# zalgo3/zfista

Hardware: AMD Instinct MI355X
Metric: fista_iterations_per_sec_n1e8_per_gpu_shard (higher is better)
Workload: dtype f64

## Files before the change

### include/zfista_hip.h

```cpp
#ifndef ZFISTA_HIP_H
#define ZFISTA_HIP_H

#include <stdint.h>

#ifdef __cplusplus
extern "C" {
#endif

#define ZF_ABI_VERSION 7

#define ZF_OK 0
#define ZF_ERR_HIP (-1)
#define ZF_ERR_ARG (-2)
#define ZF_ERR_STATE (-3)
#define ZF_ERR_NODEVICE (-4)

#define ZF_RUNNING 0
#define ZF_CONVERGED 1
#define ZF_MAXITER 2
#define ZF_BACKTRACK_FAILED 3

#define ZF_PROBLEM_DIAG_QUAD_L1 1
#define ZF_PROBLEM_LEAST_SQUARES_L1 2
#define ZF_PROBLEM_BLUR_HAAR_L1 3
// ... 71 lines not shown
    double lr;
    double tol;
    double tol_internal;
    double decay_rate;
    int64_t max_iter;
    int64_t max_backtrack_iter;
    int32_t nesterov;
    int32_t deprecated;
    int32_t sub_iters;
    int32_t accept_mode;
} zf_options;

typedef struct zf_solver zf_solver;

int zf_abi_version(void);
const char* zf_last_error(void);
int64_t zf_sizeof_control(void);
int zf_device_count(int* count);
int zf_set_device(int device);
int zf_malloc(void** dev_ptr, int64_t bytes);
int zf_free(void* dev_ptr);
int zf_memcpy_h2d(void* dst_dev, const void* src_host, int64_t bytes, void* stream);
int zf_memcpy_d2h(void* dst_host, const void* src_dev, int64_t bytes, void* stream);
int zf_memcpy_d2d(void* dst_dev, const void* src_dev, int64_t bytes, void* stream);
int zf_stream_synchronize(void* stream);
int zf_shutdown(void);

typedef struct zf_comm zf_comm;
int zf_comm_unique_id(void* id128);
int zf_comm_create(zf_comm** out, int32_t rank, int32_t world, const void* id128);
int zf_comm_destroy(zf_comm* c);
int zf_comm_create_local_group(zf_comm** out_world, int32_t world, int64_t cap_doubles);
int zf_comm_info(zf_comm* c, int32_t* rank, int32_t* world);
typedef struct zf_comm_desc {
    int32_t rank, world;
    int32_t kind;
    int32_t nccl_count;
    int32_t nccl_user_rank;
    int32_t nccl_device;
    int32_t rccl_version;
    int32_t reserved;
    int64_t all_gathers;
    char library[256];
} zf_comm_desc;
int zf_comm_describe(zf_comm* c, zf_comm_desc* out, int64_t out_bytes);
int zf_comm_all_gather(zf_comm* c, const double* send_dev, double* recv_dev, int64_t count, void* stream);

int zf_op_eval(const double* taps_dev, int32_t k, const double* b_dev, int64_t h, int64_t w, double scale,
               const double* x_host, double* f_out, double* grad_out_host);

int zf_decide_host(zf_control* ctl, int64_t ctl_bytes , const double* packs,
                   double* trace);

int zf_solver_create(zf_solver** out, const zf_problem_desc* desc, const zf_options* opt,
                     void* stream);
int zf_solver_destroy(zf_solver* s);
int zf_solver_enqueue_init(zf_solver* s, const double* x0_dev);
int zf_solver_enqueue_init_commit(zf_solver* s);
int zf_solver_set_beta(zf_solver* s, int64_t first, const double* beta_host, int64_t count);
int zf_solver_enqueue_steps(zf_solver* s, int64_t steps);
int zf_solver_autotune(zf_solver* s, int32_t* chosen_tiles);
int zf_solver_flush(zf_solver* s);
int zf_solver_set_comm(zf_solver* s, zf_comm* comm);
int zf_solver_enqueue_init_all(zf_solver* s, const double* x0_dev);
int zf_solver_enqueue_trial(zf_solver* s);
int zf_solver_enqueue_decide(zf_solver* s);
int zf_solver_sub_iters(zf_solver* s, int32_t* sub_iters);
int zf_solver_set_history(zf_solver* s, double* hist_dev, int64_t cap_slots, int64_t stride);
int zf_solver_set_max_iter(zf_solver* s, int64_t max_iter);
int zf_solver_pack_ptrs(zf_solver* s, double** pack_local_dev, double** pack_all_dev);
int zf_solver_set_pack_buffers(zf_solver* s, double* pack_local_dev, double* pack_all_dev);
int zf_solver_svec_ptrs(zf_solver* s, double** s_part_dev, double** s_all_dev);
int zf_solver_set_svec_buffers(zf_solver* s, double* s_part_dev, double* s_all_dev);
int zf_solver_enqueue_trial_finish(zf_solver* s);
int zf_solver_enqueue_init_finish(zf_solver* s);
int zf_solver_poll(zf_solver* s, zf_control* ctl_host, int64_t ctl_bytes, double* trace_host, int64_t trace_bytes);
int zf_solver_x_dev(zf_solver* s, const double** x_dev);
int zf_solver_get_x(zf_solver* s, double* x_host, int64_t count );
int zf_solver_get_x_prev(zf_solver* s, double* x_host, int64_t count );
int zf_solver_restore(zf_solver* s, const double* xk_dev, const double* xprev_dev, const zf_control* saved,
                      int64_t saved_bytes );
int zf_solver_trial_kernel_ms(zf_solver* s, double* avg_ms, int64_t* launches);
int zf_solver_launch_counts(zf_solver* s, int64_t* out, int64_t count );
int zf_solver_ls_plan(zf_solver* s, int64_t* out, int64_t count );
int zf_solver_pass_stats(zf_solver* s, double* out, int64_t count );
int zf_solver_pass_stats_ex(zf_solver* s, double* out, int64_t count );
int zf_solver_exchange_stats(zf_solver* s, double* out, int64_t count );
int zf_solver_pass_records(zf_solver* s, double* out, int64_t cap_pairs, int64_t* count);
int zf_solver_set_timing(zf_solver* s, int32_t enabled);

int zf_host_grad_step(double* v_host, const double* y_host, const double* jac_host, double lr,
                      int64_t n);
int zf_host_model_terms(const double* jac_host, const double* x_host, const double* y_host,
                        int64_t n, double out3[3]);
int zf_host_momentum(double* y_out_host, const double* x_host, const double* x_old_host,
                     double beta, int64_t n);
int zf_dev_grad_step(double* v_dev, const double* y_dev, const double* jac_dev, double lr, int64_t n, void* stream);
int zf_dev_model_terms(const double* jac_dev, const double* x_dev, const double* y_dev, int64_t n,
                       double out3_host[3], void* stream);
int zf_dev_model_terms_async(const double* jac_dev, const double* x_dev, const double* y_dev, int64_t n,
                             double* out3_dev, void* stream);
int zf_dev_momentum(double* y_out_dev, const double* x_dev, const double* x_old_dev, double beta, int64_t n,
                    void* stream);
int zf_dev_mo_combine(double* v_dev, const double* y_dev, const double* J_dev, const double* w_host, double lr,
                      int32_t m, int64_t n, double* ss_dev, void* stream);
int zf_dev_mo_post_terms(const double* J_dev, const double* y_dev, const double* p_dev, const double* v_dev,
                         int32_t m, int64_t n, double* out_dev , void* stream);

int zf_host_prox_l1_box(double* out_host, const double* x_host, double tau, double lo, double hi,
                        int64_t n);
int zf_host_asum(const double* x_host, int64_t n, double* out);
int zf_host_diag_grad(double* out_host, const double* x_host, const double* d_dev,
                      const double* c_dev, int64_t n);
int zf_ls_remainder_eval(const double* s_plus_host, const double* s_k_host, const double* s_km1_host, int64_t m, double beta,
                         int32_t nesterov, double scale, int32_t wide, double* r_out);

typedef struct zf_spmv_plan {
    int32_t lanes;
    int32_t reserved;
    int64_t threshold;
    int64_t nsplit;
    int64_t nseg;
    const int64_t* split_row;
    const int64_t* split_first;
    const int64_t* seg_start;
} zf_spmv_plan;
typedef struct zf_spmat zf_spmat;
int zf_spmat_create(zf_spmat** out, int64_t m, int64_t n, int64_t nnz, const int64_t* indptr_dev, const int32_t* indices_dev,
                    const double* values_dev, const zf_spmv_plan* plan, const int64_t* t_indptr_dev, const int32_t* t_indices_dev,
                    const double* t_values_dev, const zf_spmv_plan* t_plan, int64_t plan_bytes);
int zf_spmat_destroy(zf_spmat* h);
int zf_solver_create_sparse(zf_solver** out, const zf_problem_desc* desc, const zf_spmat* h, const zf_options* opt, void* stream);

int zf_solver_create_sparse_responses(zf_solver** out, const zf_problem_desc* desc, const zf_spmat* h, int32_t K, const zf_options* opt,
                                      void* stream);
int zf_spmat_mr_apply(const zf_spmat* h, int32_t transpose, int32_t K, double out_scale, const double* in_host, double* out_host);

int zf_solver_duality_gap(zf_solver* s, double* out, int64_t count );


int zf_solver_set_l2(zf_solver* s, double l2);
int zf_host_prox_enet_box(double* out_host, const double* x_host, double tau, double shrink, double lo, double hi, int64_t n);
int zf_host_enet_g(const double* x_host, int64_t n, double lam, double l2, double* out);

int zf_spmat_col_norms(const zf_spmat* h, double* norms_dev, double* stats_dev);
int zf_dense_col_norms(const double* A_dev, int64_t m_rows, int64_t n, double* norms_dev, double* stats_dev);
int zf_screen_scan(const uint8_t* keep_dev, int64_t n, int32_t* index_dev, int64_t* count_out);
int zf_spmat_restrict_count(const zf_spmat* h, const uint8_t* keep_dev, int32_t* index_dev, int64_t* len_dev, int64_t* t_len_dev,
                            int32_t* seg_off_dev, int64_t* count_out);
int zf_spmat_restrict_fill(const zf_spmat* h, const uint8_t* keep_dev, const int32_t* index_dev, const int32_t* seg_off_dev, int64_t k,
                           int64_t nnz_new, const int64_t* indptr_dev, int32_t* indices_dev, double* values_dev,
                           const int64_t* t_indptr_dev, int32_t* t_indices_dev, double* t_values_dev);
int zf_dense_restrict(const double* A_dev, int64_t m_rows, int64_t n, const uint8_t* keep_dev, int32_t* index_dev, int64_t k,
                      double* out_dev);

int zf_solver_set_huber(zf_solver* s, double delta);

enum { ZF_LOSS_SQUARE = 0, ZF_LOSS_LOGISTIC = 1, ZF_LOSS_HUBER = 2 };
int zf_solver_set_row_weights(zf_solver* s, const double* w_dev);

enum { ZF_LOSS_POISSON = 3 };
int zf_solver_set_poisson(zf_solver* s);

int zf_solver_set_penalty_factors(zf_solver* s, const double* p_dev);
int zf_host_prox_pf_box(double* out_host, const double* x_host, const double* p_host, double t, double lo, double hi, int64_t n);
int zf_host_pf_g(const double* x_host, const double* p_host, int64_t n, double lam, double* out);
// ... 87 lines not shown
```

### zfista_amd/_lib.py

```python
from __future__ import annotations

import ctypes as C
import os
import subprocess

import numpy as np

_HERE = os.path.dirname(os.path.abspath(__file__))
CSRC = os.path.join(_HERE, "csrc")
LIB_PATH = os.environ.get("ZF_LIB_PATH") or os.path.join(CSRC, "libzfista_hip.so")

ZF_OK = 0
ZF_RUNNING, ZF_CONVERGED, ZF_MAXITER, ZF_BACKTRACK_FAILED = 0, 1, 2, 3
ZF_PROBLEM_DIAG_QUAD_L1, ZF_PROBLEM_LEAST_SQUARES_L1, ZF_PROBLEM_BLUR_HAAR_L1 = 1, 2, 3
ZF_PROBLEM_SPARSE_LS_L1 = 4
ZF_PROBLEM_LOGISTIC_L1, ZF_PROBLEM_SPARSE_LOGISTIC_L1 = 5, 6
ZF_LOSS_SQUARE, ZF_LOSS_LOGISTIC, ZF_LOSS_HUBER, ZF_LOSS_POISSON, ZF_LOSS_MULTINOMIAL = 0, 1, 2, 3, 4
ZF_MO_GENERIC, ZF_MO_JOS1, ZF_MO_FDS = 0, 1, 2
ZF_PACK_LEN, ZF_TRACE_COLS, ZF_RING = 8, 8, 1024
ZF_MAX_SUB_ITERS = 16
ZF_MAX_LAG = 2 * ZF_MAX_SUB_ITERS - 2
ZF_PEND_FLUSH = -1
TR_ERR, TR_F, TR_LR, TR_FUN, TR_TRIALS, TR_FX, TR_GX, TR_FY = range(8)
PK_FY, PK_DOT, PK_SS, PK_GX, PK_FX, PK_ERR = range(6)
# ... 49 lines not shown
class CommDesc(C.Structure):

    _fields_ = [
        ("rank", C.c_int32), ("world", C.c_int32), ("kind", C.c_int32), ("nccl_count", C.c_int32),
        ("nccl_user_rank", C.c_int32), ("nccl_device", C.c_int32), ("rccl_version", C.c_int32), ("reserved", C.c_int32),
        ("all_gathers", C.c_int64), ("library", C.c_char * 256),
    ]


class SpmvPlan(C.Structure):

    _fields_ = [
        ("lanes", C.c_int32), ("reserved", C.c_int32), ("threshold", C.c_int64), ("nsplit", C.c_int64), ("nseg", C.c_int64),
        ("split_row", C.c_void_p), ("split_first", C.c_void_p), ("seg_start", C.c_void_p),
    ]


class EvalDesc(C.Structure):

    _fields_ = [
        ("A", C.c_void_p), ("A32", C.c_void_p), ("spmat", C.c_void_p), ("m_rows", C.c_int64), ("n", C.c_int64),
        ("b", C.c_void_p), ("w", C.c_void_p), ("p", C.c_void_p),
        ("scale", C.c_double), ("lam", C.c_double), ("l2", C.c_double), ("delta", C.c_double),
        ("loss", C.c_int32), ("K", C.c_int32),
    ]


_P = C.c_void_p
_D = C.POINTER(C.c_double)
SIGNATURES = {
    "zf_abi_version": (C.c_int, []),
    "zf_last_error": (C.c_char_p, []),
    "zf_sizeof_control": (C.c_int64, []),
    "zf_device_count": (C.c_int, [C.POINTER(C.c_int)]),
    "zf_set_device": (C.c_int, [C.c_int]),
    "zf_malloc": (C.c_int, [C.POINTER(_P), C.c_int64]),
    "zf_free": (C.c_int, [_P]),
    "zf_memcpy_h2d": (C.c_int, [_P, _P, C.c_int64, _P]),
    "zf_memcpy_d2h": (C.c_int, [_P, _P, C.c_int64, _P]),
    "zf_memcpy_d2d": (C.c_int, [_P, _P, C.c_int64, _P]),
    "zf_stream_synchronize": (C.c_int, [_P]),
    "zf_shutdown": (C.c_int, []),
    "zf_comm_unique_id": (C.c_int, [_P]),
    "zf_comm_create": (C.c_int, [C.POINTER(_P), C.c_int32, C.c_int32, _P]),
    "zf_comm_destroy": (C.c_int, [_P]),
    "zf_comm_create_local_group": (C.c_int, [C.POINTER(_P), C.c_int32, C.c_int64]),
    "zf_comm_info": (C.c_int, [_P, C.POINTER(C.c_int32), C.POINTER(C.c_int32)]),
    "zf_comm_describe": (C.c_int, [_P, C.POINTER(CommDesc), C.c_int64]),
    "zf_comm_all_gather": (C.c_int, [_P, _P, _P, C.c_int64, _P]),
    "zf_solver_set_comm": (C.c_int, [_P, _P]),
    "zf_solver_enqueue_init_all": (C.c_int, [_P, _P]),
    "zf_decide_host": (C.c_int, [C.POINTER(Control), C.c_int64, _P, _P]),
    "zf_solver_create": (C.c_int, [C.POINTER(_P), C.POINTER(ProblemDesc), C.POINTER(Options), _P]),
    "zf_solver_destroy": (C.c_int, [_P]),
    "zf_solver_enqueue_init": (C.c_int, [_P, _P]),
    "zf_solver_enqueue_init_commit": (C.c_int, [_P]),
    "zf_solver_set_beta": (C.c_int, [_P, C.c_int64, _P, C.c_int64]),
    "zf_solver_enqueue_steps": (C.c_int, [_P, C.c_int64]),
    "zf_solver_autotune": (C.c_int, [_P, C.POINTER(C.c_int32)]),
    "zf_solver_flush": (C.c_int, [_P]),
    "zf_solver_enqueue_trial": (C.c_int, [_P]),
    "zf_solver_enqueue_decide": (C.c_int, [_P]),
    "zf_solver_sub_iters": (C.c_int, [_P, C.POINTER(C.c_int32)]),
    "zf_solver_set_history": (C.c_int, [_P, _P, C.c_int64, C.c_int64]),
    "zf_solver_set_max_iter": (C.c_int, [_P, C.c_int64]),
    "zf_solver_pack_ptrs": (C.c_int, [_P, C.POINTER(_P), C.POINTER(_P)]),
    "zf_solver_set_pack_buffers": (C.c_int, [_P, _P, _P]),
    "zf_solver_svec_ptrs": (C.c_int, [_P, C.POINTER(_P), C.POINTER(_P)]),
    "zf_solver_set_svec_buffers": (C.c_int, [_P, _P, _P]),
    "zf_solver_enqueue_trial_finish": (C.c_int, [_P]),
    "zf_solver_enqueue_init_finish": (C.c_int, [_P]),
    "zf_solver_poll": (C.c_int, [_P, C.POINTER(Control), C.c_int64, _P, C.c_int64]),
    "zf_solver_x_dev": (C.c_int, [_P, C.POINTER(_P)]),
    "zf_solver_get_x": (C.c_int, [_P, _P, C.c_int64]),
    "zf_solver_get_x_prev": (C.c_int, [_P, _P, C.c_int64]),
    "zf_solver_restore": (C.c_int, [_P, _P, _P, C.POINTER(Control), C.c_int64]),
    "zf_solver_trial_kernel_ms": (C.c_int, [_P, C.POINTER(C.c_double), C.POINTER(C.c_int64)]),
    "zf_solver_set_timing": (C.c_int, [_P, C.c_int32]),
    "zf_solver_pass_stats": (C.c_int, [_P, _P, C.c_int64]),
    "zf_solver_pass_stats_ex": (C.c_int, [_P, _P, C.c_int64]),
    "zf_solver_exchange_stats": (C.c_int, [_P, _P, C.c_int64]),
    "zf_solver_pass_records": (C.c_int, [_P, _P, C.c_int64, C.POINTER(C.c_int64)]),
    "zf_solver_launch_counts": (C.c_int, [_P, _P, C.c_int64]),
    "zf_solver_ls_plan": (C.c_int, [_P, _P, C.c_int64]),
    "zf_host_grad_step": (C.c_int, [_P, _P, _P, C.c_double, C.c_int64]),
    "zf_host_model_terms": (C.c_int, [_P, _P, _P, C.c_int64, _P]),
    "zf_host_momentum": (C.c_int, [_P, _P, _P, C.c_double, C.c_int64]),
    "zf_dev_grad_step": (C.c_int, [_P, _P, _P, C.c_double, C.c_int64, _P]),
    "zf_dev_model_terms": (C.c_int, [_P, _P, _P, C.c_int64, _P, _P]),
    "zf_dev_model_terms_async": (C.c_int, [_P, _P, _P, C.c_int64, _P, _P]),
    "zf_dev_momentum": (C.c_int, [_P, _P, _P, C.c_double, C.c_int64, _P]),
    "zf_dev_mo_combine": (C.c_int, [_P, _P, _P, _P, C.c_double, C.c_int32, C.c_int64, _P, _P]),
    "zf_dev_mo_post_terms": (C.c_int, [_P, _P, _P, _P, C.c_int32, C.c_int64, _P, _P]),
    "zf_eval_diag_l1": (C.c_int, [_P, _P, _P, C.c_double, C.c_int64, _P, _P]),
    "zf_host_prox_l1_box": (C.c_int, [_P, _P, C.c_double, C.c_double, C.c_double, C.c_int64]),
    "zf_host_asum": (C.c_int, [_P, C.c_int64, C.POINTER(C.c_double)]),
    "zf_host_diag_grad": (C.c_int, [_P, _P, _P, _P, C.c_int64]),
    "zf_mo_create": (C.c_int, [C.POINTER(_P), C.c_int32, C.c_int32, C.c_int64, _P, _P, C.c_double, C.c_double, _P]),
    "zf_mo_set_shard": (C.c_int, [_P, C.c_int64, C.c_int64, _P, _P]),
    "zf_mo_set_comm": (C.c_int, [_P, _P, C.c_int64, C.c_int64]),
    "zf_mo_exchange_count": (C.c_int, [_P, C.POINTER(C.c_int64)]),
    "zf_mo_set_bounds": (C.c_int, [_P, _P, _P]),
    "zf_mo_destroy": (C.c_int, [_P]),
    "zf_mo_set_x0": (C.c_int, [_P, _P]),
    "zf_mo_eval_F": (C.c_int, [_P, C.c_int32, _P, _P]),
    "zf_mo_prepare": (C.c_int, [_P, _P]),
    "zf_mo_set_jac": (C.c_int, [_P, _P]),
    "zf_mo_dual_eval": (C.c_int, [_P, C.c_double, _P, _P]),
    "zf_mo_dual_hessian": (C.c_int, [_P, C.c_double, _P, _P]),
    "zf_mo_solve_dual": (C.c_int, [_P, C.c_double, _P, _P, C.c_int32, _P, C.c_double, C.c_int64, _P,
                                  C.POINTER(C.c_double), C.POINTER(C.c_int64), C.POINTER(C.c_int32),
                                  C.POINTER(C.c_int64)]),
    "zf_mo_solve_dual_stream": (C.c_int, [_P, C.c_double, _P, _P, C.c_int32, _P, C.c_double, C.c_int64, _P,
                                         C.POINTER(C.c_double), C.POINTER(C.c_int64), C.POINTER(C.c_int32),
                                         C.POINTER(C.c_int64)]),
    "zf_mo_solve_dual_device": (C.c_int, [_P, C.c_double, _P, _P, C.c_int32, _P, C.c_double, C.c_int64, _P,
                                         C.POINTER(C.c_double), C.POINTER(C.c_int64), C.POINTER(C.c_int32),
                                         C.POINTER(C.c_int64), C.POINTER(C.c_double), _P, _P, _P]),
    "zf_mo_prepare_async": (C.c_int, [_P]),
    "zf_mo_set_fused": (C.c_int, [_P, C.c_int32]),
    "zf_mo_trial_launch": (C.c_int, [_P, C.c_double, _P, C.c_int32, _P, C.c_double, C.c_int64, C.c_double, C.c_int32,
                                     C.c_int32, _P]),
    "zf_mo_trial_wait": (C.c_int, [_P, C.c_int32, _P, _P, _P, _P, _P, _P, _P, _P, _P, _P, _P]),
    "zf_mo_uncommit": (C.c_int, [_P]),
    "zf_mo_invalidate_prepare": (C.c_int, [_P, C.c_int32]),
    "zf_mo_debug_force_timeout": (C.c_int, [_P, C.c_int32]),
    "zf_mo_get_f_y": (C.c_int, [_P, _P]),
    "zf_mo_solve_stats": (C.c_int, [_P, _P, C.c_int64]),
    "zf_mo_recover": (C.c_int, [_P, C.c_double, _P, _P]),
    "zf_mo_commit": (C.c_int, [_P, C.c_double, C.c_int32]),
    "zf_mo_get": (C.c_int, [_P, C.c_int32, _P, C.c_int64]),
    "zf_mo_put": (C.c_int, [_P, C.c_int32, _P]),
    "zf_mo_get_jac": (C.c_int, [_P, _P, C.c_int64]),
    "zf_mo_prox_host": (C.c_int, [_P, _P, _P, _P]),
    "zf_mo_post_terms": (C.c_int, [_P, C.c_double, _P, _P, _P]),
    "zf_op_eval": (C.c_int, [_P, C.c_int32, _P, C.c_int64, C.c_int64, C.c_double, _P, C.POINTER(C.c_double), _P]),
    "zf_ls_remainder_eval": (C.c_int, [_P, _P, _P, C.c_int64, C.c_double, C.c_int32, C.c_double, C.c_int32, C.POINTER(C.c_double)]),
    "zf_spmat_create": (C.c_int, [C.POINTER(_P), C.c_int64, C.c_int64, C.c_int64, _P, _P, _P, C.POINTER(SpmvPlan),
                                  _P, _P, _P, C.POINTER(SpmvPlan), C.c_int64]),
    "zf_spmat_destroy": (C.c_int, [_P]),
    "zf_solver_duality_gap": (C.c_int, [_P, _P, C.c_int64]),
    "zf_solver_create_sparse": (C.c_int, [C.POINTER(_P), C.POINTER(ProblemDesc), _P, C.POINTER(Options), _P]),
    "zf_spmat_col_norms": (C.c_int, [_P, _P, _P]),
    "zf_dense_col_norms": (C.c_int, [_P, C.c_int64, C.c_int64, _P, _P]),
    "zf_screen_scan": (C.c_int, [_P, C.c_int64, _P, C.POINTER(C.c_int64)]),
    "zf_spmat_restrict_count": (C.c_int, [_P, _P, _P, _P, _P, _P, C.POINTER(C.c_int64)]),
    "zf_spmat_restrict_fill": (C.c_int, [_P, _P, _P, _P, C.c_int64, C.c_int64, _P, _P, _P, _P, _P, _P]),
    "zf_dense_restrict": (C.c_int, [_P, C.c_int64, C.c_int64, _P, _P, C.c_int64, _P]),
    "zf_solver_set_l2": (C.c_int, [_P, C.c_double]),
    "zf_host_prox_enet_box": (C.c_int, [_P, _P, C.c_double, C.c_double, C.c_double, C.c_double, C.c_int64]),
    "zf_host_enet_g": (C.c_int, [_P, C.c_int64, C.c_double, C.c_double, C.POINTER(C.c_double)]),
    "zf_solver_set_huber": (C.c_int, [_P, C.c_double]),
    "zf_solver_set_row_weights": (C.c_int, [_P, _P]),
    "zf_solver_set_poisson": (C.c_int, [_P]),
    "zf_solver_set_multinomial": (C.c_int, [_P]),
    "zf_solver_set_penalty_factors": (C.c_int, [_P, _P]),
    "zf_host_prox_pf_box": (C.c_int, [_P, _P, _P, C.c_double, C.c_double, C.c_double, C.c_int64]),
    "zf_host_pf_g": (C.c_int, [_P, _P, C.c_int64, C.c_double, C.POINTER(C.c_double)]),
    "zf_solver_set_matrix_f32": (C.c_int, [_P, _P]),
    "zf_solver_set_responses": (C.c_int, [_P, C.c_int32]),
    "zf_solver_create_sparse_responses": (C.c_int, [C.POINTER(_P), C.POINTER(ProblemDesc), _P, C.c_int32, C.POINTER(Options), _P]),
    "zf_spmat_mr_apply": (C.c_int, [_P, C.c_int32, C.c_int32, C.c_double, _P, _P]),
    "zf_sizeof_eval_desc": (C.c_int64, []),
    "zf_margins_eval": (C.c_int, [C.POINTER(EvalDesc), C.c_int64, _P, C.POINTER(C.c_double), _P]),
    "zf_margins_gap": (C.c_int, [C.POINTER(EvalDesc), C.c_int64, _P, _P, C.c_int64]),
    "zf_margins_screen": (C.c_int, [C.POINTER(EvalDesc), C.c_int64, _P, _P, C.c_int64, _P, _P, C.c_int64, C.c_int64, _P, _P]),
}

_lib = None


def build(verbose: bool = False) -> str:
    out = subprocess.run(["make", "-C", CSRC], capture_output=True, text=True)
    if out.returncode != 0:
        raise HipUnavailable(f"building libzfista_hip.so failed:\n{out.stdout}\n{out.stderr}")
    if verbose:
        print(out.stdout)
    return LIB_PATH


def load():
    global _lib
    if _lib is not None:
        return _lib
    if not os.path.exists(LIB_PATH):
        raise HipUnavailable(
            f"{LIB_PATH} is not built; run `make -C {CSRC}` (or __graft_entry__.build()). "
            "zfista_amd has no CPU fallback."
        )
    try:
        import torch
    except Exception:
        pass
    try:
        lib = C.CDLL(LIB_PATH)
    except OSError as exc:
        raise HipUnavailable(f"cannot load {LIB_PATH}: {exc}") from exc
    for name, (res, args) in SIGNATURES.items():
        fn = getattr(lib, name)
        fn.restype = res
        fn.argtypes = args
    if lib.zf_sizeof_control() != C.sizeof(Control):
        raise HipUnavailable("zf_control layout mismatch between library and Python mirror")
    if lib.zf_sizeof_eval_desc() != C.sizeof(EvalDesc):
        raise HipUnavailable("zf_eval_desc layout mismatch between library and Python mirror")
    _lib = lib
    return lib


def check(rc: int, what: str = ""):
    if rc != ZF_OK:
        msg = load().zf_last_error().decode(errors="replace")
        raise ZfError(f"{what or 'libzfista_hip'} failed ({rc}): {msg}")


def require_gpu():
    lib = load()
    n = C.c_int(0)
    rc = lib.zf_device_count(C.byref(n))
    if rc != ZF_OK or n.value < 1:
        raise HipUnavailable(
            "no usable GPU: " + lib.zf_last_error().decode(errors="replace")
            + " - zfista_amd runs its solver arithmetic on MI355X only (no CPU fallback)."
        )
    return lib


ENV_SWITCHES = ("ZF_SPECULATE", "ZF_LS_SMALL", "ZF_GEMV_MFMA", "ZF_TILES_PER_WG", "ZF_SUB_ITERS",
                "ZF_COMM", "ZF_MO_COMM", "ZF_MO_LAUNCH_AHEAD", "ZF_MO_SPIN_LIMIT", "ZF_RCCL_LIB", "ZF_DUAL_SOLVER",
                "ZF_FORCE_SPLIT", "ZF_LIB_PATH", "ZF_BENCH_BACKEND",
                "ZF_RUNAHEAD", "ZF_RUNAHEAD_SPIN_LIMIT", "ZF_PASS_SEQ_START", "ZF_AHEAD",
                "ZF_AHEAD_UNSHARDED", "ZF_ACCEPT", "ZF_OP_SEPARABLE", "ZF_OP_FUSE_PROX", "ZF_OP_PERSIST", "ZF_RUNAHEAD_SHARDED")


def env_overrides() -> dict:
    return {k: os.environ[k] for k in ENV_SWITCHES if k in os.environ}


def ptr(a: np.ndarray) -> int:
    return a.ctypes.data
```

### zfista_amd/csrc/zf_common.h

```cpp
#pragma once
#include <hip/hip_runtime.h>
#include <stdint.h>
#include <stdio.h>
#include <string.h>

#include "../../include/zfista_hip.h"

extern thread_local char zf_errbuf[512];
static inline int zf_fail(int code, const char* fmt, const char* a = "", const char* b = "") {
    snprintf(zf_errbuf, sizeof(zf_errbuf), fmt, a, b);
    return code;
}
#define ZF_HIP(expr)                                                                   \
    do {                                                                               \
        hipError_t _e = (expr);                                                        \
        if (_e != hipSuccess) return zf_fail(ZF_ERR_HIP, "%s: %s", #expr, hipGetErrorString(_e)); \
    } while (0)
#define ZF_REQUIRE(cond, msg)                                  \
    do {                                                       \
        if (!(cond)) return zf_fail(ZF_ERR_ARG, "%s%s", msg);  \
    } while (0)

struct zf_env {
    bool speculate;
    int pass_seq_start;
    int sub_iters;
    bool runahead;
    int tiles_per_wg;
    unsigned runahead_spin;
    int runahead_sharded;
    bool ahead;
    bool ahead_unsharded;
    bool gemv_mfma;
    bool ls_small;
    bool op_separable;
    bool op_fuse_prox;
    bool op_persist;
    long long mo_spin_limit;
};
zf_env zf_env_read();

constexpr int ZF_BLOCK = 256;
constexpr int ZF_MAX_GRID = 2048;
constexpr int ZF_WAVES = ZF_BLOCK / 64;

static inline int zf_grid_for(int64_t items_per_thread_units) {
    int64_t blocks = (items_per_thread_units + ZF_BLOCK - 1) / ZF_BLOCK;
    if (blocks < 1) blocks = 1;
    if (blocks > ZF_MAX_GRID) blocks = ZF_MAX_GRID;
    return (int)blocks;
}

__device__ __forceinline__ void zf_publish(double* p, double v) {
    __hip_atomic_store(p, v, __ATOMIC_RELAXED, __HIP_MEMORY_SCOPE_AGENT);
}
__device__ __forceinline__ double zf_consume(const double* p) {
    return __hip_atomic_load(p, __ATOMIC_RELAXED, __HIP_MEMORY_SCOPE_AGENT);
}

__device__ __forceinline__ double zf_wave_sum(double v) {
#pragma unroll
    for (int off = 32; off > 0; off >>= 1) v += __shfl_down(v, off, 64);
    return v;
}
__device__ __forceinline__ double zf_wave_max(double v) {
#pragma unroll
    for (int off = 32; off > 0; off >>= 1) v = fmax(v, __shfl_down(v, off, 64));
    return v;
}

template <int NS, int NM, int WAVES>
__device__ __forceinline__ void zf_block_reduce(const double (&sums)[NS], const double (&maxs)[NM > 0 ? NM : 1],
                                                double* lds , double& out) {
    const int lane = threadIdx.x & 63, wave = threadIdx.x >> 6;
#pragma unroll
    for (int k = 0; k < NS; ++k) {
        double v = zf_wave_sum(sums[k]);
        if (lane == 0) lds[wave * (NS + NM) + k] = v;
    }
#pragma unroll
    for (int k = 0; k < NM; ++k) {
        double v = zf_wave_max(maxs[k]);
        if (lane == 0) lds[wave * (NS + NM) + NS + k] = v;
    }
    __syncthreads();
    if (threadIdx.x < NS + NM) {
        const int k = threadIdx.x;
        double v = lds[k];
        if (k < NS) {
            for (int w = 1; w < WAVES; ++w) v += lds[w * (NS + NM) + k];
        } else {
            for (int w = 1; w < WAVES; ++w) v = fmax(v, lds[w * (NS + NM) + k]);
        }
        out = v;
    }
}

template <int N, int H, bool IS_MAX, int LVL>
__device__ __forceinline__ void zf_wave_reduce_multi_level(double (&v)[N], int lane) {
    if constexpr (LVL < 6) {
        constexpr int off = 32 >> LVL;
        if constexpr (LVL < H) {
            constexpr int half = N >> (LVL + 1);
            const bool hi = (lane & off) != 0;
#pragma unroll
            for (int q = 0; q < half; ++q) {
                const double send = hi ? v[q] : v[q + half];
                const double keep = hi ? v[q + half] : v[q];
                const double recv = __shfl_xor(send, off, 64);
                v[q] = IS_MAX ? fmax(keep, recv) : keep + recv;
            }
        } else {
            constexpr int cnt = N >> H;
#pragma unroll
            for (int q = 0; q < cnt; ++q) {
                const double recv = __shfl_xor(v[q], off, 64);
                v[q] = IS_MAX ? fmax(v[q], recv) : v[q] + recv;
            }
        }
        zf_wave_reduce_multi_level<N, H, IS_MAX, LVL + 1>(v, lane);
    }
// ... 38 lines not shown
```

### zfista_amd/csrc/zf_kernels_step.h

```cpp
#pragma once
#include <type_traits>

#include "zf_common.h"
#include "zf_decide.h"

constexpr int ZF_NPART = 6;

struct zf_elem_acc {
    double fy, dot, ss, l1, fx, mx;
};

template <bool NESTEROV, bool BOX, bool RES = false>
__device__ __forceinline__ double zf_elem_diag(double xk, double xo, double d, double c, double beta,
                                               double lr, double tau, double lo, double hi,
                                               zf_elem_acc& a) {
    double y = xk;
    if (NESTEROV) y = xk + beta * (xk - xo);
    const double r = y - c;
    const double grad = d * r;
    a.fy = __builtin_fma(grad, r, a.fy);
    const double v = y - lr * grad;
    double xn = zf_soft_threshold_nn(v, tau);
    if (BOX) xn = zf_clip(xn, lo, hi);
    const double dx = xn - y;
// ... 112 lines not shown
                     : "=&s"(keep) : "v"(gsrc), "s"(lds_dst) : "memory");
    else
        asm volatile("s_mov_b32 %0, m0\n\ts_mov_b32 m0, %2\n\ts_nop 0\n\tglobal_load_lds_dwordx4 %1, off\n\ts_mov_b32 m0, %0"
                     : "=&s"(keep) : "v"(gsrc), "s"(lds_dst) : "memory");
}
template <int N> __device__ __forceinline__ void zf_wait_vm() {
    asm volatile("s_waitcnt vmcnt(%0)" ::"n"(N) : "memory");
}
typedef __attribute__((address_space(3))) void* zf_lds_ptr;
#ifndef ZF_S16_GLDS
#define ZF_S16_GLDS 1
#endif
#ifndef ZF_S8_GLDS
#define ZF_S8_GLDS 0
#endif
#ifndef ZF_GENERAL_SINGLE_LOOP
#define ZF_GENERAL_SINGLE_LOOP 1
#endif
#ifndef ZF_GLDS_STAGES
#define ZF_GLDS_STAGES 3
#endif
#ifndef ZF_MID_REG_MAX
#define ZF_MID_REG_MAX 10
#endif
template <int S, int MODE, bool HIST, bool GRAD_INLINE, int SP = S> constexpr bool zf_uses_glds() {
    if (HIST || !GRAD_INLINE || ZF_S16_GLDS == 0) return false;
    if (S >= 16) return true;
    if (MODE == 0 && SP >= 16 && S > ZF_MID_REG_MAX) return true;
    if (ZF_S8_GLDS == 2) return S == 8 && SP >= 16 && MODE == 1;
    return ZF_S8_GLDS != 0 && S == 8 && SP >= 16;
}
constexpr int ZF_GLDS_STREAMS = 4;
constexpr int ZF_GLDS_STAGE_UNITS = ZF_GLDS_STREAMS * ZF_BLOCK;
constexpr int ZF_GLDS_NST = ZF_GLDS_STAGES;
static_assert(ZF_GLDS_NST >= 2 && ZF_GLDS_NST <= 4, "2 .. 4 stages");

constexpr int ZF_MAX_SUB = ZF_MAX_SUB_ITERS;
constexpr int zf_chain_h(int S) {
    int h = 0;
    while (h < 4 && S % (2 << h) == 0) ++h;
    return h;
}
constexpr int ZF_MID_MIN = 9;
constexpr int ZF_MID_MAX = 15;
ZF_HD inline int zf_pass_part(int S, int lag, int nf) {
    if (lag == 0 && nf == S) return 0;
#ifndef ZF_MID_CHAIN_OFF
    if (S >= 16 && lag == 0 && nf >= ZF_MID_MIN && nf <= ZF_MID_MAX) return 3;
#endif
    if (S >= 16 && nf > S / 2) return 2;
    return 1;
}
ZF_HD inline bool zf_pass_claims(int PART, int L, int S, int lag, int nf) {
    if (PART == 0) return lag == 0 && nf == S;
    if (PART == 3) return lag == 0 && nf == L;
    const bool longer = S >= 16 && nf > S / 2 && !(lag == 0 && nf == S);
    return PART == 2 ? longer : !longer && !(lag == 0 && nf == S);
}
#ifndef ZF_S16_UB
#define ZF_S16_UB 1
#endif
constexpr int ZF_MAX_RING = 6;

struct zf_pass_head {
    int cur, prev, ring;
    double lr, beta_next;
    int64_t nit;
};


struct zf_step_args {
    const zf_control* ctl;
    const double* beta_ring;
    double* xb[ZF_MAX_RING];
    const double* p0;
    const double* p1;
    double lam, lo, hi;
    int64_t n;
    int tiles_per_wg;
    double* blk_part;
    int* pass_log;
    int pass_slot;
    int pass_tag;
    double* hist;
    int64_t hist_cap;
    int64_t hist_stride;
    int fin_mode;
    int fin_gsz, fin_ng;
    double* grp_part;
    unsigned* fin_cnt;
    double fin_scale_f, fin_scale_g;
    double* pack;
    zf_control* ctl_rw;
    int decide;
    double* trace;
    int pass_seq;
    int fb_on, fb_part, fb_len;
    unsigned long long* ra_word;
    unsigned* ra_flags;
    int ra_wait;
    int ra_need;
    unsigned ra_spin;
    zf_pass_head ra_head;
    unsigned* ra_stats;
    double head_stamp;
    int head_nf;
    int fin_grid;
    int accept_mode;
};

ZF_HD inline int zf_log_shape(int lag, int nf, int passes) { return (nf & 31) | ((lag & 31) << 5) | ((passes & 63) << 10); }

struct zf_finalize_args {
    const double* blk_part;
    int nblocks;
    int sub_iters;
    double* slice_part;
    unsigned* cnt;
    double scale[ZF_NPART];
    const double* f_y_ext;
    const double* f_x_ext;
    const double* r_ext;
    int contribute_f;
    int contribute_x;
    double* pack;
    zf_control* ctl;
    int decide;
    double* trace;
    const double* beta_ring;
};

template <int S>
__global__ __launch_bounds__(ZF_FIN_THREADS) void zf_finalize_kernel(zf_finalize_args F) {
    constexpr int NQ = S * ZF_NPART;
    constexpr int NW = ZF_FIN_THREADS / 64;
    __shared__ double lds[NW * NQ];
    __shared__ zf_trial_eval s_pre[ZF_MAX_SUB_ITERS];
    __shared__ double s_pack[ZF_MAX_SUB_ITERS * ZF_PACK_LEN];
    __shared__ double s_single[NQ];
    __shared__ int s_last;
    if (F.ctl->status != ZF_RUNNING) return;
    const int lane = threadIdx.x & 63, wave = threadIdx.x >> 6;
    const int per = (F.nblocks + (int)gridDim.x - 1) / (int)gridDim.x;
    const int b0 = blockIdx.x * per;
    int b1 = b0 + per;
    if (b1 > F.nblocks) b1 = F.nblocks;
    constexpr int GT = S < 8 ? S : 8;
    constexpr int GH = zf_chain_h(GT);
#pragma unroll
    for (int j0 = 0; j0 < S; j0 += GT) {
        double sums[5 * GT], maxs[GT];
#pragma unroll
        for (int k = 0; k < 5 * GT; ++k) sums[k] = 0.0;
#pragma unroll
        for (int k = 0; k < GT; ++k) maxs[k] = 0.0;
        for (int b = b0 + threadIdx.x; b < b1; b += ZF_FIN_THREADS) {
            double p[ZF_NPART * GT];
#pragma unroll
            for (int k = 0; k < ZF_NPART * GT; ++k) p[k] = F.blk_part[(int64_t)(j0 * ZF_NPART + k) * F.nblocks + b];
#pragma unroll
            for (int j = 0; j < GT; ++j) {
#pragma unroll
                for (int k = 0; k < 5; ++k) sums[j * 5 + k] = sums[j * 5 + k] + p[j * ZF_NPART + k];
                maxs[j] = fmax(maxs[j], p[j * ZF_NPART + 5]);
            }
        }
        zf_wave_reduce_multi<5 * GT, GH, false>(sums, lane);
        zf_wave_reduce_multi<GT, GH, true>(maxs, lane);
        if ((lane & ((64 >> GH) - 1)) == 0) {
#pragma unroll
            for (int q = 0; q < 5; ++q) {
                const int idx = zf_wave_reduce_multi_index<5 * GT, GH>(q, lane);
                lds[wave * NQ + (j0 + idx / 5) * ZF_NPART + idx % 5] = sums[q];
            }
            lds[wave * NQ + (j0 + zf_wave_reduce_multi_index<GT, GH>(0, lane)) * ZF_NPART + 5] = maxs[0];
        }
    }
    __syncthreads();
    const bool single = (gridDim.x == 1);
    if (threadIdx.x < NQ) {
        const int k = threadIdx.x;
        double r = lds[k];
        for (int w = 1; w < NW; ++w)
            r = (k % ZF_NPART == ZF_NPART - 1) ? fmax(r, lds[w * NQ + k]) : r + lds[w * NQ + k];
        if (single) s_single[k] = r;
        else zf_publish(F.slice_part + (int64_t)k * ZF_FIN_WGS + blockIdx.x, r);
    }
    if (single) {
        if (threadIdx.x == 0) s_last = 1;
    } else {
        asm volatile("s_waitcnt vmcnt(0)" ::: "memory");
        if (NQ > 64) __syncthreads();
        if (threadIdx.x == 0) {
            const unsigned t = __hip_atomic_fetch_add(F.cnt, 1u, __ATOMIC_RELAXED, __HIP_MEMORY_SCOPE_AGENT);
// ... 106 lines not shown
    }
    __syncthreads();
    if (s_role == 0) return;
    auto sum_rows = [&](const double* rows, int count) -> double {
        double acc = 0.0, comp = 0.0;
        auto add = [&](double p) {
            if (is_max) {
                acc = fmax(acc, p);
            } else {
                const double tsum = acc + p;
                comp += (fabs(acc) >= fabs(p)) ? (acc - tsum) + p : (p - tsum) + acc;
                acc = tsum;
            }
        };
        if (count > 32 && count <= 64) {
            double p[64];
#pragma unroll
            for (int u = 0; u < 64; ++u) p[u] = (u < count) ? zf_consume(rows + (int64_t)u * NQ) : 0.0;
#pragma unroll
            for (int u = 0; u < 64; ++u) add(p[u]);
            return is_max ? acc : acc + comp;
        }
        for (int k0 = 0; k0 < count; k0 += 32) {
            double p[32];
#pragma unroll
            for (int u = 0; u < 32; ++u) p[u] = (k0 + u < count) ? zf_consume(rows + (int64_t)(k0 + u) * NQ) : 0.0;
#pragma unroll
            for (int u = 0; u < 32; ++u) add(p[u]);
        }
        return is_max ? acc : acc + comp;
    };
    if (s_role == 1) {
        const int g = b / gsz, b0 = g * gsz;
        const int b1 = b0 + gsz <= G ? b0 + gsz : G;
        if (t < NQ) zf_publish(A.grp_part + (int64_t)g * NQ + t, sum_rows(A.blk_part + (int64_t)b0 * NQ + t, b1 - b0));
        asm volatile("s_waitcnt vmcnt(0)" ::: "memory");
        __syncthreads();
        if (t == 0) {
            const unsigned tk = __hip_atomic_fetch_add(A.fin_cnt, 1u, __ATOMIC_RELAXED, __HIP_MEMORY_SCOPE_AGENT);
            const int last = (tk == (unsigned)(ng - 1));
            if (last) __hip_atomic_store(A.fin_cnt, 0u, __ATOMIC_RELAXED, __HIP_MEMORY_SCOPE_AGENT);
            asm volatile("s_waitcnt vmcnt(0)" ::: "memory");
            s_role = last ? 2 : 0;
        }
        __syncthreads();
        if (s_role != 2) return;
    }
    if (t < NQ) s_tot[t] = grouped ? sum_rows(A.grp_part + t, ng) : sum_rows(A.blk_part + t, G);
    __syncthreads();
    if (t >= 64) return;
    constexpr int SH = zf_chain_h(SP);
    constexpr int LSTR = 64 >> SH;
    const int trial = t / LSTR;
    const double* q = s_tot + trial * ZF_NPART;
    double pk[ZF_PACK_LEN];
    pk[ZF_PK_FY] = A.fin_scale_f * q[0];
    pk[ZF_PK_DOT] = q[1];
    pk[ZF_PK_SS] = q[2];
    pk[ZF_PK_GX] = A.fin_scale_g * q[3];
    pk[ZF_PK_FX] = A.fin_scale_f * q[4];
    pk[ZF_PK_ERR] = q[5];
    pk[7] = 0.0;
    if (A.accept_mode != 0) {
        pk[7] = pk[ZF_PK_FX];
        pk[ZF_PK_FX] = pk[ZF_PK_FY] + pk[7];
    }
    pk[6] = A.decide ? 0.0 : zf_pack_stamp(A.ctl_rw);
    if constexpr (RA) {
        if (!A.decide) {
            const bool poisoned = __hip_atomic_load(A.ra_flags + G + (A.pass_seq & 3), __ATOMIC_RELAXED, __HIP_MEMORY_SCOPE_AGENT) == (unsigned)A.pass_seq;
            pk[6] = poisoned ? 0.0 : A.head_stamp;
        }
    }
    if (t % LSTR == 0) {
#pragma unroll
        for (int k = 0; k < ZF_PACK_LEN; ++k) {
            A.pack[trial * ZF_PACK_LEN + k] = pk[k];
            s_pack[trial * ZF_PACK_LEN + k] = pk[k];
        }
    }
    if constexpr (RA) {
        if (!A.decide) {
            if (t == 0 && A.pass_log) A.pass_log[A.pass_slot] = A.pass_tag | zf_log_shape(0, LEN, 0);
            return;
        }
        constexpr int CW = (int)(sizeof(zf_control) / 8);
        static_assert(sizeof(zf_control) % 8 == 0 && CW <= 64, "one lane per word of the control block");
        unsigned long long* gw = reinterpret_cast<unsigned long long*>(const_cast<zf_control*>(A.ctl));
        unsigned long long* lw = reinterpret_cast<unsigned long long*>(A.ctl_rw);
        unsigned long long W = __hip_atomic_load(A.ra_word, __ATOMIC_RELAXED, __HIP_MEMORY_SCOPE_AGENT);
        int ok = 1;
        if (A.ra_wait != 0) {
            for (unsigned k = 0; (int)(W >> 32) < A.ra_wait && k < A.ra_spin; ++k) {
                __builtin_amdgcn_s_sleep(2);
                W = __hip_atomic_load(A.ra_word, __ATOMIC_RELAXED, __HIP_MEMORY_SCOPE_AGENT);
            }
            ok = ((int)(W >> 32) >= A.ra_wait && (int)(unsigned)W >= A.ra_wait) ? 1 : 0;
            if (t == 0 && (int)(W >> 32) < A.ra_wait) __hip_atomic_fetch_add(A.ra_stats + 0, 1u, __ATOMIC_RELAXED, __HIP_MEMORY_SCOPE_AGENT);
        }
        if (__hip_atomic_load(A.ra_flags + G + (A.pass_seq & 3), __ATOMIC_RELAXED, __HIP_MEMORY_SCOPE_AGENT) == (unsigned)A.pass_seq) ok = 0;
        zf_control* c = A.ctl_rw;
        if (ok) {
            if (t < CW) lw[t] = __hip_atomic_load(gw + t, __ATOMIC_RELAXED, __HIP_MEMORY_SCOPE_AGENT);
            __builtin_amdgcn_wave_barrier();
            ok = (c->status == ZF_RUNNING && c->pend_status == 0 && c->lag == 0 && c->nit == A.ra_head.nit &&
                  c->lr == A.ra_head.lr && c->cur == A.ra_head.cur && c->prev == A.ra_head.prev && zf_fresh_len(c) == LEN) ? 1 : 0;
        }
        ok = __builtin_amdgcn_readfirstlane(ok);
        unsigned good = (unsigned)W;
        if (ok) {
            zf_decide_pass_wave(c, s_pack, pk, A.trace, A.beta_ring, t, LSTR, s_pre);
            if (t == 0) c->pass_seq = A.pass_seq;
            __builtin_amdgcn_wave_barrier();
            if (t < CW) __hip_atomic_store(gw + t, lw[t], __ATOMIC_RELAXED, __HIP_MEMORY_SCOPE_AGENT);
            if (c->status == ZF_RUNNING && c->pend_status == 0 && c->lag == 0 && c->nit == A.ra_head.nit + LEN && c->lr == A.ra_head.lr)
                good = (unsigned)A.pass_seq;
        }
        if (t == 0) {
            if (A.pass_log) A.pass_log[A.pass_slot] = A.pass_tag | (ok ? zf_log_shape(0, LEN, 0) : 0);
            if (!ok) __hip_atomic_fetch_add(A.ra_stats + 1, 1u, __ATOMIC_RELAXED, __HIP_MEMORY_SCOPE_AGENT);
        }
        asm volatile("s_waitcnt vmcnt(0)" ::: "memory");
        if (t == 0)
            __hip_atomic_store(A.ra_word, ((unsigned long long)(unsigned)A.pass_seq << 32) | good, __ATOMIC_RELAXED, __HIP_MEMORY_SCOPE_AGENT);
        return;
    }
    if (A.decide) {
        zf_decide_pass_wave(A.ctl_rw, s_pack, pk, A.trace, A.beta_ring, t, LSTR, s_pre);
        if (t == 0) A.ctl_rw->pass_seq = A.pass_seq;
    }
}

struct zf_ahead_check {
    zf_pass_head head;
    int nf;
    int seq;
};
__device__ __forceinline__ void zf_decide_ahead(zf_control* ctl, const double* packs, const double (&pk)[ZF_PACK_LEN], double* trace,
                                                const double* beta_ring, int lane, int lstr, zf_trial_eval* lds_pre,
                                                const zf_ahead_check& H, bool packs_ok, unsigned long long* ra_word,
                                                unsigned* ra_stats, int* pass_log, int pass_slot, int pass_tag) {
    const unsigned long long W = __hip_atomic_load(ra_word, __ATOMIC_RELAXED, __HIP_MEMORY_SCOPE_AGENT);
    unsigned good = (unsigned)W;
    const bool ok = packs_ok && ctl->status == ZF_RUNNING && ctl->pend_status == 0 && ctl->lag == 0 && ctl->nit == H.head.nit &&
                    ctl->lr == H.head.lr && ctl->cur == H.head.cur && ctl->prev == H.head.prev && zf_fresh_len(ctl) == H.nf;
    if (ok) {
        zf_decide_pass_wave(ctl, packs, pk, trace, beta_ring, lane, lstr, lds_pre);
        if (lane == 0) ctl->pass_seq = H.seq;
        __builtin_amdgcn_wave_barrier();
        if (ctl->status == ZF_RUNNING && ctl->pend_status == 0 && ctl->lag == 0 && ctl->nit == H.head.nit + H.nf && ctl->lr == H.head.lr)
            good = (unsigned)H.seq;
    } else if (lane == 0) {
        __hip_atomic_fetch_add(ra_stats + 2, 1u, __ATOMIC_RELAXED, __HIP_MEMORY_SCOPE_AGENT);
        if (pass_log) pass_log[pass_slot] = pass_tag;
    }
    if (lane == 0)
        __hip_atomic_store(ra_word, ((unsigned long long)(unsigned)H.seq << 32) | good, __ATOMIC_RELAXED, __HIP_MEMORY_SCOPE_AGENT);
}

template <int SP>
__global__ __launch_bounds__(128) void zf_tail_kernel(zf_step_args A) {
    constexpr int NQ = SP * ZF_NPART;
    static_assert(NQ <= 128, "one thread per row value");
    __shared__ int s_last;
    __shared__ double s_tot[NQ];
    __shared__ double s_pack[ZF_MAX_SUB_ITERS * ZF_PACK_LEN];
    __shared__ zf_trial_eval s_pre[ZF_MAX_SUB_ITERS];
    const int t = (int)threadIdx.x, G = A.fin_grid, g = (int)blockIdx.x;
    const int gsz = A.fin_gsz, ng = A.fin_ng;
    const bool grouped = gsz > 1;
    const bool is_max = (t % ZF_NPART == ZF_NPART - 1);
    if (grouped) {
        const int b0 = g * gsz;
        const int b1 = b0 + gsz <= G ? b0 + gsz : G;
        if (t < NQ) zf_publish(A.grp_part + (int64_t)g * NQ + t, zf_sum_rows<NQ>(A.blk_part + (int64_t)b0 * NQ + t, b1 - b0, is_max));
        asm volatile("s_waitcnt vmcnt(0)" ::: "memory");
        __syncthreads();
        if (t == 0) {
            const unsigned tk = __hip_atomic_fetch_add(A.fin_cnt, 1u, __ATOMIC_RELAXED, __HIP_MEMORY_SCOPE_AGENT);
            const int last = (tk == (unsigned)(ng - 1));
            if (last) __hip_atomic_store(A.fin_cnt, 0u, __ATOMIC_RELAXED, __HIP_MEMORY_SCOPE_AGENT);
            asm volatile("s_waitcnt vmcnt(0)" ::: "memory");
            s_last = last;
        }
        __syncthreads();
        if (!s_last) return;
    }
    if (t < NQ) s_tot[t] = grouped ? zf_sum_rows<NQ>(A.grp_part + t, ng, is_max) : zf_sum_rows<NQ>(A.blk_part + t, G, is_max);
    __syncthreads();
    if (t >= 64) return;
    constexpr int SH = zf_chain_h(SP);
    constexpr int LSTR = 64 >> SH;
    const int trial = t / LSTR;
    const double* q = s_tot + trial * ZF_NPART;
    double pk[ZF_PACK_LEN];
    pk[ZF_PK_FY] = A.fin_scale_f * q[0];
    pk[ZF_PK_DOT] = q[1];
    pk[ZF_PK_SS] = q[2];
    pk[ZF_PK_GX] = A.fin_scale_g * q[3];
    pk[ZF_PK_FX] = A.fin_scale_f * q[4];
    pk[ZF_PK_ERR] = q[5];
    pk[7] = 0.0;
    if (A.accept_mode != 0) {
        pk[7] = pk[ZF_PK_FX];
        pk[ZF_PK_FX] = pk[ZF_PK_FY] + pk[7];
    }
    pk[6] = A.decide ? 0.0 : A.head_stamp;
    if (t % LSTR == 0) {
#pragma unroll
        for (int k = 0; k < ZF_PACK_LEN; ++k) {
            A.pack[trial * ZF_PACK_LEN + k] = pk[k];
            s_pack[trial * ZF_PACK_LEN + k] = pk[k];
        }
    }
    if (A.decide) {
        zf_ahead_check H;
        H.head = A.ra_head;
        H.nf = A.head_nf;
        H.seq = A.pass_seq;
        zf_decide_ahead(A.ctl_rw, s_pack, pk, A.trace, A.beta_ring, t, LSTR, s_pre, H, true, A.ra_word, A.ra_stats, A.pass_log,
                        A.pass_slot, A.pass_tag);
    }
}

__device__ __forceinline__ unsigned long long zf_uniform_u64(unsigned long long v) {
    const unsigned lo = __builtin_amdgcn_readfirstlane((unsigned)v);
    const unsigned hi = __builtin_amdgcn_readfirstlane((unsigned)(v >> 32));
    return ((unsigned long long)hi << 32) | lo;
}
__device__ __forceinline__ double zf_uniform_f64(double v) {
    return __longlong_as_double((long long)zf_uniform_u64((unsigned long long)__double_as_longlong(v)));
}
__device__ __forceinline__ double zf_readlane_f64(double v, int i) {
    const long long b = __double_as_longlong(v);
    const unsigned lo = (unsigned)__builtin_amdgcn_readlane((int)(unsigned)b, i);
    const unsigned hi = (unsigned)__builtin_amdgcn_readlane((int)(unsigned)(b >> 32), i);
    return __longlong_as_double((long long)(((unsigned long long)hi << 32) | lo));
}
__device__ __forceinline__ zf_pass_head zf_head_of(const zf_control* c) {
    zf_pass_head h;
    h.cur = c->cur;
    h.prev = c->prev;
    h.ring = c->ring_size;
    h.lr = c->lr;
    h.beta_next = c->beta_next;
    h.nit = c->nit;
    return h;
}

template <bool GRAD_INLINE, bool NESTEROV, bool BOX, bool NT, int S, int MODE, bool HIST, int SP = S, bool COH = false, bool RES = false,
          bool ENET = false, bool PF = false>
__device__ __forceinline__ double zf_trial_body(const zf_step_args& A, double* lds, const zf_pass_head& HD, const int lag,
                                                const int nf, zf_d2* stage = nullptr, const double l2 = 0.0) {
    constexpr bool FULL = (MODE == 0);
    static_assert(!RES || GRAD_INLINE, "resolved differences f(x+) - f(y): the separable problem");
    static_assert(!ENET || (!GRAD_INLINE && S == 1 && MODE == 0 && !COH), "elastic net: single trials on a gradient vector");
    static_assert(!PF || (!GRAD_INLINE && S == 1 && MODE == 0 && !COH && !ENET && NT), "penalty factors: single trials on a gradient vector");
    static_assert(!COH || (FULL && !HIST && GRAD_INLINE && SP >= 16 && ZF_S16_GLDS != 0),
                  "coherent iterate traffic: branch-free chains of a 16-chain solver through the DMA pipeline");
    constexpr bool GLDS = COH || zf_uses_glds<S, MODE, HIST, GRAD_INLINE, SP>();
    const unsigned tidx = threadIdx.x;
    constexpr bool FRESH_FULL = (MODE <= 1);
    const int cur = HD.cur;
    const int prev = HD.prev;
    const int ring = HD.ring;
    const double lr = HD.lr;
    const int ntr = FULL ? S : (FRESH_FULL ? lag + S : lag + nf);
    double beta[S];
    const int64_t nit = HD.nit;
    const int64_t base = nit - lag;
    beta[0] = NESTEROV ? ((FULL || lag == 0) ? HD.beta_next : A.beta_ring[nit % ZF_RING]) : 0.0;
#pragma unroll
    for (int j = 1; j < S; ++j)
        beta[j] = NESTEROV ? (COH ? zf_uniform_f64(A.beta_ring[(nit + j) % ZF_RING]) : A.beta_ring[(nit + j) % ZF_RING]) : 0.0;
    const double tau = A.lam * lr;
    double shrink = 1.0, hl2 = 0.0;
    if constexpr (ENET) {
        shrink = 1.0 / (1.0 + l2 * lr);
        hl2 = 0.5 * l2;
    }
    double rp_lr = 0.0, rp_beta = 0.0, rp_tau = 0.0;
    if constexpr (!FULL && GRAD_INLINE) {
        const int rl = (int)(tidx & 63);
        if (rl < lag) {
            rp_lr = A.ctl->lag_lr[rl];
            rp_beta = NESTEROV ? A.beta_ring[(base + rl) % ZF_RING] : 0.0;
            rp_tau = A.lam * rp_lr;
        }
    }
    auto replay_param = [&](int i, double& b_i, double& lr_i, double& tau_i) {
        b_i = zf_readlane_f64(rp_beta, i);
        lr_i = zf_readlane_f64(rp_lr, i);
        tau_i = zf_readlane_f64(rp_tau, i);
    };
    int first, second;
    zf_free_bufs(cur, prev, ring, &first, &second);
    const double* __restrict__ xk = A.xb[cur];
    const double* __restrict__ xo = A.xb[prev];
    double* __restrict__ out_last = A.xb[ntr == 1 ? first : second];
    double* __restrict__ out_prev = A.xb[first];
    const double* __restrict__ p0 = A.p0;
    const double* __restrict__ p1 = A.p1;
    const int64_t n = A.n;

    zf_elem_acc acc[S];
#pragma unroll
    for (int j = 0; j < S; ++j) acc[j] = {0.0, 0.0, 0.0, 0.0, 0.0, 0.0};
    const int64_t n2 = n >> 1;
    const zf_d2* __restrict__ xk2 = reinterpret_cast<const zf_d2*>(xk);
    const zf_d2* __restrict__ xo2 = reinterpret_cast<const zf_d2*>(xo);
    const zf_d2* __restrict__ p02 = reinterpret_cast<const zf_d2*>(p0);
    const zf_d2* __restrict__ p12 = reinterpret_cast<const zf_d2*>(p1);

    auto advance = [&](zf_d2 a, zf_d2 o, zf_d2 q, zf_d2 cc, int64_t i) {
#pragma unroll
        for (int j = 0; j < S; ++j) {
            if (FRESH_FULL || j < nf) {
                zf_d2 r;
                if (GRAD_INLINE) {
                    r.x = zf_elem_diag<NESTEROV, BOX, RES>(a.x, o.x, q.x, cc.x, beta[j], lr, tau, A.lo, A.hi, acc[j]);
                    r.y = zf_elem_diag<NESTEROV, BOX, RES>(a.y, o.y, q.y, cc.y, beta[j], lr, tau, A.lo, A.hi, acc[j]);
                } else if constexpr (ENET) {
                    r.x = zf_elem_vec_enet<NESTEROV, BOX>(a.x, o.x, q.x, beta[j], lr, tau, shrink, A.lam, hl2, A.lo, A.hi, acc[j]);
                    r.y = zf_elem_vec_enet<NESTEROV, BOX>(a.y, o.y, q.y, beta[j], lr, tau, shrink, A.lam, hl2, A.lo, A.hi, acc[j]);
                } else if constexpr (PF) {
                    r.x = zf_elem_vec_pf<NESTEROV, BOX>(a.x, o.x, q.x, cc.x, beta[j], lr, tau, A.lo, A.hi, acc[j]);
                    r.y = zf_elem_vec_pf<NESTEROV, BOX>(a.y, o.y, q.y, cc.y, beta[j], lr, tau, A.lo, A.hi, acc[j]);
                } else {
                    r.x = zf_elem_vec<NESTEROV, BOX>(a.x, o.x, q.x, beta[j], lr, tau, A.lo, A.hi, acc[j]);
                    r.y = zf_elem_vec<NESTEROV, BOX>(a.y, o.y, q.y, beta[j], lr, tau, A.lo, A.hi, acc[j]);
                }
                o = a;
                a = r;
                if (HIST)
                    zf_st2<NT>(reinterpret_cast<zf_d2*>(A.hist + ((nit + j + 1) % A.hist_cap) * A.hist_stride) + i, a);
            }
        }
        if constexpr (COH) {
            zf_st2_coh(reinterpret_cast<zf_d2*>(out_last) + i, a);
            zf_st2_coh(reinterpret_cast<zf_d2*>(out_prev) + i, o);
        } else {
            zf_st2<NT>(reinterpret_cast<zf_d2*>(out_last) + i, a);
            if (S > 1 && (FRESH_FULL || ntr >= 2)) zf_st2<NT>(reinterpret_cast<zf_d2*>(out_prev) + i, o);
        }
        if (S >= 8) __builtin_amdgcn_sched_barrier(0);
    };

    const int64_t full_tiles = n2 / ZF_TILE_UNITS;
    const int64_t G = gridDim.x;
    const int full_tiles32 = (int)full_tiles, G32 = (int)gridDim.x, b32 = (int)blockIdx.x;
#ifndef ZF_M1_UB
#define ZF_M1_UB ZF_TILE_U
#endif
    constexpr int UB = (S >= 16) ? ZF_S16_UB : (S >= 8) ? ((MODE == 1 && S == 8 && !HIST) ? ZF_M1_UB : ZF_S8_UB) : ZF_TILE_U;
    auto load_batch = [&](int64_t first_unit, zf_d2 (&a)[UB], zf_d2 (&o)[UB], zf_d2 (&q)[UB], zf_d2 (&cc)[UB]) {
#pragma unroll
        for (int u = 0; u < UB; ++u) {
            const int64_t i = first_unit + u * ZF_BLOCK;
            a[u] = zf_ld2<NT && (ZF_X_NT != 0) && (S > 1)>(xk2 + i);
            o[u] = a[u];
            if (NESTEROV) o[u] = zf_ld2<NT && (ZF_X_NT != 0) && (S > 1)>(xo2 + i);
            q[u] = zf_ld2<NT>(p02 + i);
            cc[u] = q[u];
            if (GRAD_INLINE || PF) cc[u] = zf_ld2<NT>(p12 + i);
        }
        __builtin_amdgcn_sched_barrier(0);
    };
    auto compute_batch = [&](int64_t first_unit, zf_d2 (&a)[UB], zf_d2 (&o)[UB], zf_d2 (&q)[UB], zf_d2 (&cc)[UB]) {
        if constexpr (!FULL && GRAD_INLINE) {
            for (int i = 0; i < lag; ++i) {
                double b_i, lr_i, tau_i;
                replay_param(i, b_i, lr_i, tau_i);
#pragma unroll
                for (int u = 0; u < UB; ++u) {
                    zf_d2 r;
                    r.x = zf_elem_diag_replay<NESTEROV, BOX>(a[u].x, o[u].x, q[u].x, cc[u].x, b_i, lr_i, tau_i, A.lo, A.hi);
                    r.y = zf_elem_diag_replay<NESTEROV, BOX>(a[u].y, o[u].y, q[u].y, cc[u].y, b_i, lr_i, tau_i, A.lo, A.hi);
// ... 189 lines not shown
                if (S > 1 && (FRESH_FULL || ntr >= 2)) out_prev[e] = o;
            }
        }
    }

    constexpr int RS = S + (S > 1 ? (S & 1) : 0);
    constexpr int H = zf_chain_h(RS);
    constexpr int NQ = S * ZF_NPART;
    const int lane = tidx & 63, wave = tidx >> 6;
    double sums[5 * RS], maxs[RS];
#pragma unroll
    for (int j = 0; j < RS; ++j) {
        if (j < S) {
            sums[j * 5 + 0] = acc[j].fy;
            sums[j * 5 + 1] = acc[j].dot;
            sums[j * 5 + 2] = acc[j].ss;
            sums[j * 5 + 3] = acc[j].l1;
            sums[j * 5 + 4] = acc[j].fx;
            maxs[j] = acc[j].mx;
        } else {
#pragma unroll
            for (int k = 0; k < 5; ++k) sums[j * 5 + k] = 0.0;
            maxs[j] = 0.0;
        }
    }
    zf_wave_reduce_multi<5 * RS, H, false>(sums, lane);
    zf_wave_reduce_multi<RS, H, true>(maxs, lane);
    if ((lane & ((64 >> H) - 1)) == 0) {
#pragma unroll
        for (int q = 0; q < ((5 * RS) >> H); ++q) {
            const int idx = zf_wave_reduce_multi_index<5 * RS, H>(q, lane);
            if (idx / 5 < S) lds[wave * NQ + (idx / 5) * ZF_NPART + idx % 5] = sums[q];
        }
#pragma unroll
        for (int q = 0; q < (RS >> H); ++q) {
            const int tr = zf_wave_reduce_multi_index<RS, H>(q, lane);
            if (tr < S) lds[wave * NQ + tr * ZF_NPART + 5] = maxs[q];
        }
    }
    __syncthreads();
    double v = 0.0;
    if (tidx < NQ) {
        const int t = tidx;
        v = lds[t];
#pragma unroll
        for (int w = 1; w < ZF_WAVES; ++w) v = (t % ZF_NPART == 5) ? fmax(v, lds[w * NQ + t]) : v + lds[w * NQ + t];
    }
    return v;
}

template <int SP>
__device__ __forceinline__ void zf_pass_finish(const zf_step_args& A, const double v) {
    if (A.fin_mode == 0) {
        if (threadIdx.x < SP * ZF_NPART) A.blk_part[(int64_t)threadIdx.x * gridDim.x + blockIdx.x] = v;
        return;
    }
    zf_pass_tail<SP>(A, v);
}

__device__ __forceinline__ void zf_first_pass_left(unsigned long long* ra_word, int pass_seq) {
    __hip_atomic_store(ra_word + 1, (unsigned long long)(unsigned)pass_seq, __ATOMIC_RELAXED, __HIP_MEMORY_SCOPE_AGENT);
    const unsigned long long W = __hip_atomic_load(ra_word, __ATOMIC_RELAXED, __HIP_MEMORY_SCOPE_AGENT);
    __hip_atomic_store(ra_word, ((unsigned long long)(unsigned)pass_seq << 32) | (unsigned)W, __ATOMIC_RELEASE, __HIP_MEMORY_SCOPE_AGENT);
}

__device__ __forceinline__ void zf_count_second_behind_left(unsigned long long* ra_word, unsigned* ra_stats, int ra_wait) {
    __builtin_amdgcn_fence(__ATOMIC_ACQUIRE, "agent");
    if (__hip_atomic_load(ra_word + 1, __ATOMIC_RELAXED, __HIP_MEMORY_SCOPE_AGENT) == (unsigned long long)(unsigned)ra_wait)
        __hip_atomic_fetch_add(ra_stats + 3, 1u, __ATOMIC_RELAXED, __HIP_MEMORY_SCOPE_AGENT);
}

template <bool GRAD_INLINE, bool NESTEROV, bool BOX, bool NT, int S, bool HIST = false, int PART = 0, int L = 0, bool AHEAD = false,
          bool RES = false>
__global__ __launch_bounds__(ZF_BLOCK) void zf_trial_kernel(zf_step_args A) {
    static_assert(GRAD_INLINE || S == 1, "temporal blocking needs an elementwise gradient");
    static_assert(PART <= 1 || S >= 16, "the third and fourth kernels exist for chains of 16 only");
    static_assert(PART != 3 || (L >= ZF_MID_MIN && L <= ZF_MID_MAX), "mid chains: ZF_MID_MIN .. ZF_MID_MAX trials");
    static_assert(!AHEAD || (S >= 16 && !HIST && (PART == 0 || PART == 3)), "passes ahead: full and mid chains of a 16-chain solver");
    __shared__ double lds[ZF_WAVES * S * ZF_NPART];
    constexpr bool GLDS = PART == 3 ? zf_uses_glds<(PART == 3 ? L : S), 0, HIST, GRAD_INLINE, S>()
                          : PART != 1 ? zf_uses_glds<S, PART == 0 ? 0 : 2, HIST, GRAD_INLINE>()
                                      : (S >= 16 && zf_uses_glds<S / 2, 1, HIST, GRAD_INLINE, S>());
    __shared__ zf_d2 stage[GLDS ? ZF_GLDS_NST * ZF_GLDS_STAGE_UNITS : 1];
    if constexpr (AHEAD) {
        if (A.ra_need != 0) {
            const unsigned long long W = __hip_atomic_load(A.ra_word, __ATOMIC_RELAXED, __HIP_MEMORY_SCOPE_AGENT);
            if ((int)(unsigned)W < A.ra_need) return;
        } else if (A.ra_wait == 0) {
            const zf_control* c = A.ctl;
            constexpr int LEN0 = PART == 3 ? L : S;
            const zf_pass_head& q = A.ra_head;
            if (!(c->status == ZF_RUNNING && c->pend_status == 0 && c->lag == 0 && c->nit == q.nit && c->lr == q.lr && c->cur == q.cur &&
                  c->prev == q.prev && zf_fresh_len(c) == LEN0)) {
                if (blockIdx.x == 0 && threadIdx.x == 0) zf_first_pass_left(A.ra_word, A.pass_seq);
                return;
            }
        } else {
            const unsigned long long W = __hip_atomic_load(A.ra_word, __ATOMIC_RELAXED, __HIP_MEMORY_SCOPE_AGENT);
            if ((int)(W >> 32) >= A.ra_wait && (int)(unsigned)W < A.ra_wait) {
                if (blockIdx.x == 0 && threadIdx.x == 0) zf_count_second_behind_left(A.ra_word, A.ra_stats, A.ra_wait);
                return;
            }
        }
        zf_pass_head HA = A.ra_head;
        HA.beta_next = NESTEROV ? A.beta_ring[HA.nit % ZF_RING] : 0.0;
        constexpr int LEN = PART == 3 ? L : S;
        if (A.pass_log && blockIdx.x == 0 && threadIdx.x == 0) A.pass_log[A.pass_slot] = A.pass_tag | zf_log_shape(0, LEN, 0);
        const double va = zf_trial_body<GRAD_INLINE, NESTEROV, BOX, NT, LEN, 0, HIST, S, false, RES>(A, lds, HA, 0, LEN, stage);
        if (threadIdx.x < S * ZF_NPART) A.blk_part[(int64_t)blockIdx.x * (S * ZF_NPART) + threadIdx.x] = va;
        return;
    }
    if (A.ctl->status != ZF_RUNNING) return;
    if (A.fin_mode != 0 && A.decide && A.ctl->pass_seq == A.pass_seq) return;
    const zf_pass_head HD = zf_head_of(A.ctl);
    if constexpr (S == 1) {
        if (A.pass_log && blockIdx.x == 0 && threadIdx.x == 0) A.pass_log[A.pass_slot] = A.pass_tag | zf_log_shape(0, 1, 0);
        zf_pass_finish<S>(A, zf_trial_body<GRAD_INLINE, NESTEROV, BOX, NT, S, 0, HIST, S, false, RES>(A, lds, HD, 0, 1));
    } else {
        const int lag = A.ctl->lag;
        const int nf = zf_fresh_len(A.ctl);
        if constexpr (PART == 2) {
            if (A.fb_on ? (A.fb_part >= 0 && zf_pass_claims(A.fb_part, A.fb_len, S, lag, nf)) : !zf_pass_claims(2, 0, S, lag, nf)) return;
        } else {
            if (!zf_pass_claims(PART, L, S, lag, nf)) return;
        }
        if (A.pass_log && blockIdx.x == 0 && threadIdx.x == 0) A.pass_log[A.pass_slot] = A.pass_tag | zf_log_shape(lag, nf, 0);
        double v;
        if constexpr (PART == 0) {
            v = zf_trial_body<GRAD_INLINE, NESTEROV, BOX, NT, S, 0, HIST, S, false, RES>(A, lds, HD, 0, S, stage);
        } else if constexpr (PART == 3) {
            v = zf_trial_body<GRAD_INLINE, NESTEROV, BOX, NT, L, 0, HIST, S, false, RES>(A, lds, HD, 0, L, stage);
        } else if constexpr (PART == 2) {
            const int nf_opaque = __builtin_amdgcn_readfirstlane(nf);
            v = zf_trial_body<GRAD_INLINE, NESTEROV, BOX, NT, S, 2, HIST, S, false, RES>(A, lds, HD, lag, nf_opaque, stage);
        } else if constexpr (S >= 16) {
            constexpr int SS = S / 2;
            if (lag == 0 && nf == SS) v = zf_trial_body<GRAD_INLINE, NESTEROV, BOX, NT, SS, 0, HIST, S, false, RES>(A, lds, HD, 0, SS, stage);
            else if (nf == SS) v = zf_trial_body<GRAD_INLINE, NESTEROV, BOX, NT, SS, 1, HIST, S, false, RES>(A, lds, HD, lag, SS, stage);
            else v = zf_trial_body<GRAD_INLINE, NESTEROV, BOX, NT, SS, 2, HIST, S, false, RES>(A, lds, HD, lag, nf, stage);
        } else {
            if (nf == S) v = zf_trial_body<GRAD_INLINE, NESTEROV, BOX, NT, S, 1, HIST, S, false, RES>(A, lds, HD, lag, S);
            else v = zf_trial_body<GRAD_INLINE, NESTEROV, BOX, NT, S, 2, HIST, S, false, RES>(A, lds, HD, lag, nf);
        }
        zf_pass_finish<S>(A, v);
    }
}

template <bool NESTEROV, bool BOX, bool HIST>
__global__ __launch_bounds__(ZF_BLOCK) void zf_trial_enet_kernel(zf_step_args A, double l2) {
    __shared__ double lds[ZF_WAVES * ZF_NPART];
    if (A.ctl->status != ZF_RUNNING) return;
    const zf_pass_head HD = zf_head_of(A.ctl);
    if (A.pass_log && blockIdx.x == 0 && threadIdx.x == 0) A.pass_log[A.pass_slot] = A.pass_tag | zf_log_shape(0, 1, 0);
    const double v = zf_trial_body<false, NESTEROV, BOX, true, 1, 0, HIST, 1, false, false, true>(A, lds, HD, 0, 1, nullptr, l2);
    if (threadIdx.x < ZF_NPART) A.blk_part[(int64_t)threadIdx.x * gridDim.x + blockIdx.x] = v;
}

template <bool NESTEROV, bool BOX, bool HIST>
__global__ __launch_bounds__(ZF_BLOCK) void zf_trial_pf_kernel(zf_step_args A) {
    __shared__ double lds[ZF_WAVES * ZF_NPART];
    if (A.ctl->status != ZF_RUNNING) return;
    const zf_pass_head HD = zf_head_of(A.ctl);
    if (A.pass_log && blockIdx.x == 0 && threadIdx.x == 0) A.pass_log[A.pass_slot] = A.pass_tag | zf_log_shape(0, 1, 0);
    const double v = zf_trial_body<false, NESTEROV, BOX, true, 1, 0, HIST, 1, false, false, false, true>(A, lds, HD, 0, 1);
    if (threadIdx.x < ZF_NPART) A.blk_part[(int64_t)threadIdx.x * gridDim.x + blockIdx.x] = v;
}

template <bool NESTEROV, bool BOX, bool NT, bool RES = false, int L = 0>
__global__ __launch_bounds__(ZF_BLOCK) __attribute__((amdgpu_waves_per_eu(2, 2))) void zf_runahead_kernel(zf_step_args A) {
    constexpr int S = ZF_MAX_SUB;
    static_assert(S == 16, "run-ahead passes are chains of a 16-chain solver");
    static_assert(L == 0 || (L >= ZF_MID_MIN && L <= ZF_MID_MAX), "a full chain, or a mid chain of ZF_MID_MIN .. ZF_MID_MAX trials");
    constexpr int LEN = L == 0 ? S : L;
    __shared__ double lds[ZF_WAVES * S * ZF_NPART];
    __shared__ zf_d2 stage[ZF_GLDS_NST * ZF_GLDS_STAGE_UNITS];
    __shared__ zf_control s_ctl;
    __shared__ int s_go;
    zf_pass_head HD = A.ra_head;
    const int b = (int)blockIdx.x, G = (int)gridDim.x;
    if (A.ra_wait == 0) {
        const zf_control* c = A.ctl;
        const bool same = c->status == ZF_RUNNING && c->pend_status == 0 && c->lag == 0 && c->nit == HD.nit && c->lr == HD.lr &&
                          c->cur == HD.cur && c->prev == HD.prev && zf_fresh_len(c) == LEN;
        if (!same) {
            if (b == 0 && threadIdx.x == 0) {
                zf_first_pass_left(A.ra_word, A.pass_seq);
                __hip_atomic_fetch_add(A.ra_stats + 1, 1u, __ATOMIC_RELAXED, __HIP_MEMORY_SCOPE_AGENT);
            }
            return;
        }
    } else {
        if (threadIdx.x == 0) {
            int go = 1;
            unsigned long long W = __hip_atomic_load(A.ra_word, __ATOMIC_RELAXED, __HIP_MEMORY_SCOPE_AGENT);
            if (A.ra_need != 0 && (int)(unsigned)W < A.ra_need) {
                go = 0;
            } else {
                unsigned k = 0;
                for (;;) {
                    if (A.ra_spin != 0 && (int)__hip_atomic_load(A.ra_flags + b, __ATOMIC_RELAXED, __HIP_MEMORY_SCOPE_AGENT) >= A.ra_wait) break;
                    if ((k & 15) == 15) {
                        W = __hip_atomic_load(A.ra_word, __ATOMIC_RELAXED, __HIP_MEMORY_SCOPE_AGENT);
                        if ((int)(W >> 32) >= A.ra_wait && (int)(unsigned)W < A.ra_wait) {
                            if (A.ra_need == 0 && b == 0) zf_count_second_behind_left(A.ra_word, A.ra_stats, A.ra_wait);
                            go = 2;
                            break;
                        }
                    }
                    if (++k > A.ra_spin) {
                        __hip_atomic_store(A.ra_flags + G + (A.pass_seq & 3), (unsigned)A.pass_seq, __ATOMIC_RELAXED, __HIP_MEMORY_SCOPE_AGENT);
                        __hip_atomic_fetch_add(A.ra_stats + 0, 1u, __ATOMIC_RELAXED, __HIP_MEMORY_SCOPE_AGENT);
                        go = 2;
                        break;
                    }
                    __builtin_amdgcn_s_sleep(2);
                }
            }
            s_go = go;
        }
        __syncthreads();
    }
    const int go = A.ra_wait == 0 ? 1 : __builtin_amdgcn_readfirstlane(s_go);
    if (go == 0) {
        if (b == 0 && threadIdx.x == 0) __hip_atomic_fetch_add(A.ra_stats + 1, 1u, __ATOMIC_RELAXED, __HIP_MEMORY_SCOPE_AGENT);
        return;
    }
    const bool run = go == 1;
    HD.beta_next = NESTEROV ? zf_uniform_f64(A.beta_ring[HD.nit % ZF_RING]) : 0.0;
    double v = 0.0;
    if (run) v = zf_trial_body<true, NESTEROV, BOX, NT, LEN, 0, false, S, true, RES>(A, lds, HD, 0, LEN, stage);
    zf_step_args T = A;
    T.ctl = A.ctl_rw;
    T.ctl_rw = &s_ctl;
    zf_pass_tail<S, true, LEN>(T, v);
}

template <bool GRAD_INLINE, bool BOX>
__global__ __launch_bounds__(ZF_BLOCK) void zf_eval_kernel(const double* __restrict__ x,
                                                           const double* __restrict__ d,
                                                           const double* __restrict__ c, double lo,
                                                           double hi, int64_t n, double* partials) {
    __shared__ double lds[ZF_WAVES * 3];
    double f = 0.0, l1 = 0.0, viol = 0.0;
    const int64_t stride = (int64_t)gridDim.x * ZF_BLOCK;
    for (int64_t i = (int64_t)blockIdx.x * ZF_BLOCK + threadIdx.x; i < n; i += stride) {
        const double xv = x[i];
        if (GRAD_INLINE) {
            const double r = xv - c[i];
            f += d[i] * (r * r);
        }
        l1 += fabs(xv);
        if (BOX) viol += (xv < lo || xv > hi) ? 1.0 : 0.0;
    }
    const double sums[3] = {f, l1, viol};
    const double maxs[1] = {0.0};
    double out = 0.0;
    zf_block_reduce<3, 0, ZF_WAVES>(sums, maxs, lds, out);
    if (threadIdx.x < 3) partials[(int64_t)threadIdx.x * gridDim.x + blockIdx.x] = out;
}

constexpr int ZF_FIN_BLOCK = 256;
__device__ __forceinline__ void zf_finalize_partials(const double* __restrict__ partials, int nblocks,
                                                     int nq, int max_index, double* lds ,
                                                     double* totals ) {
    const int lane = threadIdx.x & 63, wave = threadIdx.x >> 6;
    constexpr int W = ZF_FIN_BLOCK / 64;
    for (int k = 0; k < nq; ++k) {
        const bool is_max = (k == max_index);
        double v = 0.0;
        for (int b = threadIdx.x; b < nblocks; b += ZF_FIN_BLOCK) {
            const double p = partials[(int64_t)k * nblocks + b];
            v = is_max ? fmax(v, p) : v + p;
        }
        v = is_max ? zf_wave_max(v) : zf_wave_sum(v);
        if (lane == 0) lds[wave * 8 + k] = v;
    }
    __syncthreads();
    if (threadIdx.x < nq) {
        const int k = threadIdx.x;
        double v = lds[k];
        for (int w = 1; w < W; ++w) v = (k == max_index) ? fmax(v, lds[w * 8 + k]) : v + lds[w * 8 + k];
        totals[k] = v;
    }
    __syncthreads();
}
```

### zfista_amd/csrc/zf_solver.hip

```cpp
#include <algorithm>
#include <cstring>
#include <map>
#include <mutex>
#include <new>
#include <tuple>
#include <vector>

#include "zf_common.h"
#include "zf_decide.h"
#include "zf_kernels_gemv.h"
#include "zf_kernels_ls_small.h"
#include "zf_kernels_gemv_f32.h"
#include "zf_kernels_mr.h"
#include "zf_kernels_op.h"
#include "zf_spmv.h"
#include "zf_matview.h"
#include "zf_screen.h"
#include "zf_kernels_loss.h"
#include "zf_kernels_gap.h"
#include "zf_kernels_softmax.h"
#include "zf_loss_dispatch.h"
#include "zf_kernels_step.h"
#include "zf_solver_options.h"
#include "zf_trial_launch.h"

thread_local char zf_errbuf[512] = "";

#define ZF_KEEP_FIRST(expr)                                                       \
    do {                                                                          \
        hipError_t _e = (expr);                                                   \
        if (_e != hipSuccess && rc == ZF_OK)                                      \
            rc = zf_fail(ZF_ERR_HIP, "%s: %s", #expr, hipGetErrorString(_e));     \
    } while (0)

__global__ __launch_bounds__(ZF_BLOCK) void zf_sum_parts_kernel(const zf_control* ctl, const double* __restrict__ s_all,
                                                                int world, int64_t m, zf_ring3 sr, int slot) {
    int idx = 0;
    if (slot >= 0) {
        if (ctl->status != ZF_RUNNING) return;
        idx = (ctl->cur + slot) % 3;
    }
    double* __restrict__ out = sr.p[idx];
    const int64_t stride = (int64_t)gridDim.x * ZF_BLOCK;
    for (int64_t i = (int64_t)blockIdx.x * ZF_BLOCK + threadIdx.x; i < m; i += stride) {
        double t = s_all[i];
        for (int r = 1; r < world; ++r) t += s_all[(int64_t)r * m + i];
        out[i] = t;
    }
}

__global__ __launch_bounds__(64) void zf_decide_kernel(zf_control* ctl, const double* packs, double* trace,
                                                       const double* beta_ring, int sub, int stamped) {
    __shared__ zf_trial_eval s_pre[ZF_MAX_SUB_ITERS];
    if (blockIdx.x != 0) return;
    const int lane = threadIdx.x;
    if (stamped != 0) {
        const double want = zf_pack_stamp(ctl);
        const int world = ctl->world;
        for (int r = 0; r < world; ++r)
            if (packs[(int64_t)r * sub * ZF_PACK_LEN + 6] != want) return;
    }
    double pk[ZF_PACK_LEN] = {0.0, 0.0, 0.0, 0.0, 0.0, 0.0, 0.0, 0.0};
    if (lane < sub) zf_reduce_packs(packs + lane * ZF_PACK_LEN, ctl->world, sub * ZF_PACK_LEN, pk);
    zf_decide_pass_wave(ctl, packs, pk, trace, beta_ring, lane, 1, s_pre);
}

__global__ __launch_bounds__(64) void zf_decide_ahead_kernel(zf_control* ctl, const double* packs, double* trace, const double* beta_ring,
                                                             int sub, zf_ahead_check H, unsigned long long* ra_word, unsigned* ra_stats,
                                                             int* pass_log, int pass_slot, int pass_tag) {
    __shared__ zf_trial_eval s_pre[ZF_MAX_SUB_ITERS];
    if (blockIdx.x != 0) return;
    const int lane = threadIdx.x;
    bool packs_ok = true;
    {
        const double want = zf_pack_stamp(ctl);
        const int world = ctl->world;
        for (int r = 0; r < world; ++r)
            if (packs[(int64_t)r * sub * ZF_PACK_LEN + 6] != want) packs_ok = false;
    }
    double pk[ZF_PACK_LEN] = {0.0, 0.0, 0.0, 0.0, 0.0, 0.0, 0.0, 0.0};
    if (lane < sub) zf_reduce_packs(packs + lane * ZF_PACK_LEN, ctl->world, sub * ZF_PACK_LEN, pk);
    zf_decide_ahead(ctl, packs, pk, trace, beta_ring, lane, 1, s_pre, H, packs_ok, ra_word, ra_stats, pass_log, pass_slot, pass_tag);
}
// ... 127 lines not shown
    bool own_svec = true;
    bool initialised = false;
    bool init_enqueued = false;
    bool own_packs = true;
    zf_solver_options o;
    bool small_shape = false;
    bool mfma_shape = false;
    const zf_spmat* sp = nullptr;
    zf_sweep_ws ws = {nullptr, 1, 0, nullptr, nullptr};
    bool loss_part = false;
    double* gap_xp = nullptr;
    zf_op_plan op_plan = {};
    double* op_buf = nullptr;
    const double* op_taps = nullptr, *op_sep = nullptr;
    double* row_part = nullptr;
    unsigned* ls_cnt = nullptr;
    int64_t ntiles = 1;
    int tiles = 1;
    int max_grid = 1;
    bool timing = false;
    std::vector<std::pair<hipEvent_t, hipEvent_t>> ev_pool;
    size_t ev_used = 0;
    double ms_total = 0.0;
    int64_t ms_count = 0;
    std::vector<std::pair<int, float>> records;
    std::vector<std::pair<hipEvent_t, hipEvent_t>> xev_pool;
    size_t xev_used = 0;
    double xms_total = 0.0;
    int64_t xms_count = 0;
    int* pass_log = nullptr;
    int64_t launches = 0;
    int64_t first_uncollected = 0;
    double ms_full = 0.0, ms_part = 0.0;
    int64_t n_full = 0, n_part = 0;
    int64_t fresh_part = 0, lag_part = 0;
    zf_comm* comm = nullptr;
    int part_mask = 7;
    int mid_len = 0;
    int fb_part = -1, fb_len = 0;
    int64_t steps_issued = 0, kernels_issued = 0;
    int pass_seq = 0;
    zf_control shadow;
    bool shadow_valid = false;
    bool careful = false;
    int64_t steps_since_poll = 0;
    int64_t polled_rejections = 0;
    bool ra = false;
    int ra_cap = -1;
    int ra_cap_mid[ZF_MAX_SUB_ITERS] = {};
    hipStream_t stream2 = nullptr;
    hipStream_t stream3 = nullptr;
    hipEvent_t ra_join3 = nullptr;
    bool ra_c_pending = false;
    bool chunk_last = false;
    bool ra_sharded = true;
    int64_t ras_passes = 0;
    hipEvent_t ra_join = nullptr;
    hipEvent_t ra_fork = nullptr;
    bool ra_b_pending = false;
    bool ra_fork_due = false;
    int ra_last = 0, ra_last2 = 0;
    int ra_last_idx = 0;
    zf_pass_head ra_last_head = {};
    unsigned long long* ra_word = nullptr;
    unsigned* ra_flags = nullptr;
    double* blk_part2 = nullptr;
    double* grp_part2 = nullptr;
    unsigned* fin_cnt2 = nullptr;
    double* pack2 = nullptr;
    int64_t ra_passes = 0, ra_ahead = 0;
    unsigned* ra_stats = nullptr;
    int64_t ra_timeouts = 0, ra_voids = 0, ah_voids = 0, second_voids = 0;
    bool ra_off = false;
    bool ah = false;
    bool ah_unsharded = false;
    hipEvent_t ah_evT[4] = {}, ah_evD[4] = {};
    int ah_run = 0;
    int ah_last_nf = 0;
    int run_mode = 0;
    int64_t ah_passes = 0;
    double* hist = nullptr;
    int64_t hist_cap = 0, hist_stride = 0;
    zf_gap_ws gap = {nullptr, nullptr, nullptr, nullptr};
};
constexpr int ZF_PASS_LOG = 4096;
constexpr size_t ZF_CTL_SLOT = (sizeof(zf_control) + 255) / 256 * 256;
constexpr size_t ZF_STATS_OFF = ZF_CTL_SLOT - 32;
static_assert(sizeof(zf_control) <= ZF_STATS_OFF, "the run-ahead counters live behind the control block, inside its slot");
constexpr size_t ZF_TRACE_BYTES = sizeof(double) * ZF_RING * ZF_TRACE_COLS;
constexpr size_t ZF_MAIL_BYTES = ZF_CTL_SLOT + ZF_TRACE_BYTES + sizeof(int) * ZF_PASS_LOG;

static int zf_tiles_for(int64_t ntiles);
constexpr bool ZF_AHEAD_UNSHARDED_DEFAULT = false;

zf_env zf_env_read() {
    zf_env v;
    const char* e;
    v.speculate = !((e = getenv("ZF_SPECULATE")) && atoi(e) == 0);
    v.pass_seq_start = (e = getenv("ZF_PASS_SEQ_START")) ? (int)std::min<long long>(std::max<long long>(atoll(e), 0), 0x7ffffff0LL) : 0;
    v.sub_iters = (e = getenv("ZF_SUB_ITERS")) ? atoi(e) : 0;
    v.runahead = !((e = getenv("ZF_RUNAHEAD")) && atoi(e) == 0);
    v.tiles_per_wg = (e = getenv("ZF_TILES_PER_WG")) ? std::max(1, atoi(e)) : 0;
    v.runahead_spin = (e = getenv("ZF_RUNAHEAD_SPIN_LIMIT")) ? (unsigned)strtoul(e, nullptr, 10) : 1u << 13;
    v.runahead_sharded = (e = getenv("ZF_RUNAHEAD_SHARDED")) ? (atoi(e) != 0 ? 1 : 0) : -1;
    v.ahead = !((e = getenv("ZF_AHEAD")) && atoi(e) == 0);
    v.ahead_unsharded = (e = getenv("ZF_AHEAD_UNSHARDED")) ? atoi(e) != 0 : ZF_AHEAD_UNSHARDED_DEFAULT;
    v.gemv_mfma = !((e = getenv("ZF_GEMV_MFMA")) && atoi(e) == 0);
    v.ls_small = !((e = getenv("ZF_LS_SMALL")) && atoi(e) == 0);
    v.op_separable = !((e = getenv("ZF_OP_SEPARABLE")) && atoi(e) == 0);
    v.op_fuse_prox = !((e = getenv("ZF_OP_FUSE_PROX")) && atoi(e) == 0);
    v.op_persist = !((e = getenv("ZF_OP_PERSIST")) && atoi(e) == 0);
    v.mo_spin_limit = (e = getenv("ZF_MO_SPIN_LIMIT")) ? atoll(e) : 0;
    return v;
}

static int zf_solver_free_all(zf_solver* s) {
    if (s->stream2) (void)hipStreamDestroy(s->stream2);
    if (s->stream3) (void)hipStreamDestroy(s->stream3);
    if (s->ra_join3) (void)hipEventDestroy(s->ra_join3);
    for (int k = 0; k < 4; ++k) {
        if (s->ah_evT[k]) (void)hipEventDestroy(s->ah_evT[k]);
        if (s->ah_evD[k]) (void)hipEventDestroy(s->ah_evD[k]);
    }
    if (s->ra_join) (void)hipEventDestroy(s->ra_join);
    if (s->ra_fork) (void)hipEventDestroy(s->ra_fork);
    void* ptrs[] = {s->ws.part_A, s->ws.part_At, s->op_buf, s->row_part, s->ls_cnt, s->blk_part, s->slice_part, s->fin_cnt, s->grp_part, s->xbuf, s->partials, s->ctl_trace, s->beta_ring,
                    s->ra_word, s->ra_flags, s->blk_part2, s->grp_part2, s->fin_cnt2, s->pack2,
                    s->own_packs ? s->pack_local : nullptr, s->own_packs ? s->pack_all : nullptr,
                    s->grad, s->sbuf, s->resid, s->ws.slab, s->ls_scal, s->gap.rvec, s->gap.g, s->gap.part, s->gap.scal, s->gap_xp,
                    s->own_svec ? s->s_part : nullptr, s->own_svec ? s->s_all : nullptr};
    for (void* p : ptrs)
        if (p) (void)hipFree(p);
    if (s->mail) (void)hipHostFree(s->mail);
    for (auto& e : s->ev_pool) {
        (void)hipEventDestroy(e.first);
        (void)hipEventDestroy(e.second);
    }
    for (auto& e : s->xev_pool) {
        (void)hipEventDestroy(e.first);
        (void)hipEventDestroy(e.second);
    }
    return ZF_OK;
}

static zf_trial_sel zf_sel_of(const zf_solver* s) { return zf_trial_sel{s->opt.nesterov != 0, s->box, s->res}; }

static bool zf_aligned16(const void* p) { return (reinterpret_cast<uintptr_t>(p) & 15u) == 0; }

static bool zf_is_ls(int kind) {
    return kind == ZF_PROBLEM_LEAST_SQUARES_L1 || kind == ZF_PROBLEM_BLUR_HAAR_L1 || kind == ZF_PROBLEM_SPARSE_LS_L1;
}
static bool zf_is_logistic(int kind) { return kind == ZF_PROBLEM_LOGISTIC_L1 || kind == ZF_PROBLEM_SPARSE_LOGISTIC_L1; }
static bool zf_is_dense_mat(int kind) { return kind == ZF_PROBLEM_LEAST_SQUARES_L1 || kind == ZF_PROBLEM_LOGISTIC_L1; }
static bool zf_is_sparse_mat(int kind) { return kind == ZF_PROBLEM_SPARSE_LS_L1 || kind == ZF_PROBLEM_SPARSE_LOGISTIC_L1; }
static bool zf_has_margins(int kind) { return zf_is_ls(kind) || zf_is_logistic(kind); }
static_assert(ZF_OPT_MAX_K == ZF_MR_MAX_K && ZF_OPT_MAX_K == ZF_SPMM_MAX_K, "one bound of the response count");
static zf_options_base zf_base_of(const zf_solver* s) {
    const zf_problem_desc& d = s->desc;
    return zf_options_base{(int)d.kind, (int)d.world, s->accept_mode, s->init_enqueued || s->initialised, d.m_rows, d.n, d.b, s->small_shape, s->mfma_shape};
}
static zf_loss zf_loss_of(const zf_solver* s) { return zf_loss{zf_options_loss(s->desc.kind, s->o), s->o.huber, s->o.roww, s->o.K}; }
static zf_matview zf_mat_of(const zf_solver* s, const zf_solver_options& o) {
    const zf_options_view v = zf_options_view_of(zf_base_of(s), o);
    return zf_matview{v.f32 ? nullptr : s->desc.A, v.m, v.n, s->sp, s->sp != nullptr, o.A32, v.K, v.mfma};
}
static zf_matview zf_mat_of(const zf_solver* s) { return zf_mat_of(s, s->o); }
static bool zf_small_open(const zf_solver* s) { return zf_options_small_open(zf_base_of(s), s->o); }
static double zf_g_scale(const zf_solver* s) { return zf_options_g_is_whole(s->o) ? 1.0 : s->desc.lam; }
static zf_op_args zf_op_of(const zf_problem_desc& d, const zf_control* ctl, const zf_op_plan& pl, const double* taps, const double* sep) {
    zf_op_args P;
    P.ctl = ctl;
    P.H = (int)d.op_h;
    P.W = (int)d.op_w;
    P.K = pl.K;
    P.taps = taps;
    P.sep = pl.sep ? sep : nullptr;
    P.tiles = pl.grid;
    return P;
}
static zf_op_args zf_op_of(const zf_solver* s, const zf_control* ctl) { return zf_op_of(s->desc, ctl, s->op_plan, s->op_taps, s->op_sep); }
static zf_op_fuse zf_op_no_fuse() {
    zf_op_fuse F;
    memset(&F, 0, sizeof(F));
    return F;
}
constexpr int64_t ZF_OP_FUSE_MAX_PIXELS = int64_t(5) << 20;
static int zf_op_prepare(const zf_env& env, const double* taps_dev, int k, int64_t h, int64_t w, hipStream_t st, zf_op_plan* pl,
                         double** buf, const double** taps_out, const double** sep_out) {
    double host[ZF_OP_MAXK * ZF_OP_MAXK];
    ZF_HIP(hipMemcpyAsync(host, taps_dev, sizeof(double) * k * k, hipMemcpyDeviceToHost, st));
    ZF_HIP(hipStreamSynchronize(st));
    const int K = k < 3 ? 3 : k;
    double up[ZF_OP_MAXK * ZF_OP_MAXK + 2 * (ZF_OP_MAXK + 1)];
    memset(up, 0, sizeof(up));
    const int pad = (K - k) / 2;
// ... 112 lines not shown
            delete s;
            return zf_fail(ZF_ERR_ARG, "zf_solver_create: accept_mode must be ZF_ACCEPT_REFERENCE, ZF_ACCEPT_RESOLVED for "
                                       "ZF_PROBLEM_DIAG_QUAD_L1 (the element-wise difference f(x+) - f(y) exists for the separable problem only), or "
                                       "ZF_ACCEPT_REMAINDER for ZF_PROBLEM_LEAST_SQUARES_L1 and ZF_PROBLEM_SPARSE_LS_L1 (the Taylor remainder "
                                       "scale |A (x+ - y)|^2 is formed by the least-squares residual kernels only)%s");
        }
        s->accept_mode = opt->accept_mode;
        s->res = res_ok;
        s->rem = rem_ok;
    }
    const int64_t n = desc->n;
    const int64_t n_pad = (n + 63) & ~int64_t(63);
    {
        int64_t ntiles = (n / 2 + ZF_TILE_UNITS - 1) / ZF_TILE_UNITS;
        if (ntiles < 1) ntiles = 1;
        if (ntiles > 0x7fffffff) {
            delete s;
            return zf_fail(ZF_ERR_ARG, "zf_solver_create: n too large for one rank");
        }
        s->ntiles = ntiles;
        s->grid = (int)ntiles;
        s->max_grid = s->grid;
    }
#define ZF_TRY(expr)                                                                    \
    do {                                                                                \
        hipError_t _e = (expr);                                                         \
        if (_e != hipSuccess) {                                                         \
            zf_solver_free_all(s);                                                      \
            delete s;                                                                   \
            return zf_fail(ZF_ERR_HIP, "%s: %s", #expr, hipGetErrorString(_e));         \
        }                                                                               \
    } while (0)
    if (desc->kind == ZF_PROBLEM_DIAG_QUAD_L1) {
        int sub = opt->sub_iters;
        if (sub <= 0) sub = s->env.sub_iters;
        if (sub <= 0) sub = ZF_DEFAULT_SUB_ITERS;
        if (sub > ZF_MAX_SUB) sub = ZF_MAX_SUB;
        s->sub = sub >= 16 ? 16 : sub >= 8 ? 8 : sub >= 4 ? 4 : sub >= 2 ? 2 : 1;
        if (s->res && s->sub != 16) s->sub = 1;
    }
    s->ring = s->sub > 1 ? 4 : 3;
    {
        const int t = s->env.tiles_per_wg > 0 ? s->env.tiles_per_wg : zf_tiles_for(s->ntiles);
        const int64_t grid = (s->ntiles + t - 1) / t;
        const bool chains16 = desc->kind == ZF_PROBLEM_DIAG_QUAD_L1 && s->sub >= 16;
        s->ra = s->env.runahead && chains16;
        if (s->env.runahead_sharded >= 0) s->ra_sharded = s->env.runahead_sharded != 0;
        if (s->ra) {
            s->ra_cap = zf_runahead_capacity(zf_sel_of(s), s->sub);
            s->ra = grid <= s->ra_cap;
            for (int l = 0; l < ZF_MAX_SUB_ITERS; ++l) s->ra_cap_mid[l] = -1;
        }
        s->ah = s->env.ahead && chains16;
        s->ah_unsharded = s->ah && desc->world == 1 && s->env.ahead_unsharded;
    }
    if (s->ra || (s->ah && (desc->world > 1 || s->ah_unsharded))) {
        s->ring = 6;
        if (zf_second_stream(s) != hipSuccess) {
            (void)hipGetLastError();
            s->ra = false;
            s->ah = false;
        }
    }
    ZF_TRY(hipMalloc(&s->xbuf, sizeof(double) * s->ring * n_pad));
    for (int k = 0; k < s->ring; ++k) s->xb[k] = s->xbuf + k * n_pad;
    ZF_TRY(hipMalloc(&s->partials, sizeof(double) * ZF_NPART * ZF_MAX_GRID));
    {
        int64_t parts = std::max<int64_t>(s->max_grid, n / LS_SMALL_COLS + 1);
        if (desc->kind == ZF_PROBLEM_BLUR_HAAR_L1)
            parts = std::max<int64_t>(parts, zf_op_make_plan(desc->op_h, desc->op_w, (int)desc->op_k, false, false).grid);
        ZF_TRY(hipMalloc(&s->blk_part, sizeof(double) * ZF_NPART * s->sub * parts));
    }
    ZF_TRY(hipMalloc(&s->slice_part, sizeof(double) * ZF_NPART * s->sub * ZF_FIN_WGS));
    ZF_TRY(hipMalloc(&s->fin_cnt, sizeof(unsigned) * ZF_FIN_CNT_STRIDE * (ZF_FIN_GROUPS + 2)));
    ZF_TRY(hipMemsetAsync(s->fin_cnt, 0, sizeof(unsigned) * ZF_FIN_CNT_STRIDE * (ZF_FIN_GROUPS + 2), s->stream));
    ZF_TRY(hipMalloc(&s->grp_part, sizeof(double) * ZF_NPART * s->sub * ZF_FIN_GROUPS));
    ZF_TRY(hipMalloc(&s->ctl_trace, ZF_MAIL_BYTES));
    s->ctl = reinterpret_cast<zf_control*>(s->ctl_trace);
    s->trace = reinterpret_cast<double*>(s->ctl_trace + ZF_CTL_SLOT);
    s->pass_log = reinterpret_cast<int*>(s->ctl_trace + ZF_CTL_SLOT + ZF_TRACE_BYTES);
    s->ra_stats = reinterpret_cast<unsigned*>(s->ctl_trace + ZF_STATS_OFF);
    ZF_TRY(hipMemsetAsync(s->ctl_trace, 0, ZF_CTL_SLOT, s->stream));
    ZF_TRY(hipMemsetAsync(s->pass_log, 0xff, sizeof(int) * ZF_PASS_LOG, s->stream));
    ZF_TRY(hipHostMalloc(&s->mail, ZF_MAIL_BYTES, hipHostMallocDefault));
    ZF_TRY(hipMalloc(&s->beta_ring, sizeof(double) * ZF_RING));
    ZF_TRY(hipMalloc(&s->pack_local, sizeof(double) * ZF_PACK_LEN * s->sub));
    ZF_TRY(hipMalloc(&s->pack_all, sizeof(double) * ZF_PACK_LEN * s->sub * desc->world));
    ZF_TRY(hipMemsetAsync(s->trace, 0, sizeof(double) * ZF_RING * ZF_TRACE_COLS, s->stream));
    ZF_TRY(hipMemsetAsync(s->beta_ring, 0, sizeof(double) * ZF_RING, s->stream));
    ZF_TRY(hipMemsetAsync(s->pack_all, 0, sizeof(double) * ZF_PACK_LEN * s->sub * desc->world, s->stream));
    if (zf_has_margins(desc->kind)) {
        const int64_t m_pad = (desc->m_rows + 63) & ~int64_t(63);
        ZF_TRY(hipMalloc(&s->grad, sizeof(double) * n_pad));
        ZF_TRY(hipMalloc(&s->sbuf, sizeof(double) * 3 * m_pad));
        for (int k = 0; k < 3; ++k) s->sring.p[k] = s->sbuf + k * m_pad;
        ZF_TRY(hipMalloc(&s->resid, sizeof(double) * m_pad));
        ZF_TRY(hipMalloc(&s->ls_scal, sizeof(double) * 8));
    }
    if (desc->kind == ZF_PROBLEM_BLUR_HAAR_L1) {
        if (zf_op_prepare(s->env, desc->op_taps, (int)desc->op_k, desc->op_h, desc->op_w, s->stream, &s->op_plan, &s->op_buf, &s->op_taps, &s->op_sep) != ZF_OK) {
            zf_solver_free_all(s);
            delete s;
            return ZF_ERR_HIP;
        }
        ZF_TRY(hipMalloc(&s->row_part, sizeof(double) * 2 * s->op_plan.grid));
        ZF_TRY(hipMemsetAsync(s->row_part, 0, sizeof(double) * 2 * s->op_plan.grid, s->stream));
        ZF_TRY(hipMalloc(&s->ls_cnt, 64));
        ZF_TRY(hipMemsetAsync(s->ls_cnt, 0, 64, s->stream));
    }
    if (zf_is_sparse_mat(desc->kind)) {
        if (sp->A.nseg > 0) ZF_TRY(hipMalloc(&s->ws.part_A, sizeof(double) * sp->A.nseg * K));
        if (sp->At.nseg > 0) ZF_TRY(hipMalloc(&s->ws.part_At, sizeof(double) * sp->At.nseg * K));
        ZF_TRY(hipMalloc(&s->row_part, sizeof(double) * 3 * ZF_SPMV_RESID_MAX_CHUNKS));
    }
    if (zf_is_dense_mat(desc->kind)) {
        const int64_t m = desc->m_rows;
        zf_view_slices(zf_mat_of(s), &s->ws.slices, &s->ws.rows_per_slice);
        ZF_TRY(hipMalloc(&s->ws.slab, sizeof(double) * s->ws.slices * n));
        if (desc->world > 1) {
            const int64_t len = desc->row_sharded ? n : m;
            ZF_TRY(hipMalloc(&s->s_part, sizeof(double) * ((len + 63) & ~int64_t(63))));
            ZF_TRY(hipMalloc(&s->s_all, sizeof(double) * len * desc->world));
        }
        s->small_shape = desc->kind == ZF_PROBLEM_LEAST_SQUARES_L1 && desc->world == 1 && n % LS_SMALL_COLS == 0 && m <= LS_SMALL_MAX_M &&
                         m * n <= LS_SMALL_MAX_ELEMS && zf_aligned16(desc->A) && s->env.ls_small;
        if (s->small_shape) {
            ZF_TRY(hipMalloc(&s->row_part, sizeof(double) * 2 * ((m + ZF_WAVES - 1) / ZF_WAVES)));
            ZF_TRY(hipMalloc(&s->ls_cnt, 64));
            ZF_TRY(hipMemsetAsync(s->ls_cnt, 0, 64, s->stream));
        }
        if (desc->kind == ZF_PROBLEM_LOGISTIC_L1)
            ZF_TRY(hipMalloc(&s->row_part, sizeof(double) * 2 * ZF_SPMV_RESID_MAX_CHUNKS));
    }
#undef ZF_TRY
    *out = s;
    return ZF_OK;
}

extern "C" int zf_solver_create(zf_solver** out, const zf_problem_desc* desc, const zf_options* opt, void* stream) {
    return zf_solver_create_impl(out, desc, opt, stream, nullptr);
}

extern "C" int zf_solver_create_sparse(zf_solver** out, const zf_problem_desc* desc, const zf_spmat* h, const zf_options* opt, void* stream) {
    ZF_REQUIRE(out && desc && h && opt, "zf_solver_create_sparse: null argument");
    ZF_REQUIRE(zf_is_sparse_mat(desc->kind), "zf_solver_create_sparse: desc->kind must be ZF_PROBLEM_SPARSE_LS_L1 or ZF_PROBLEM_SPARSE_LOGISTIC_L1");
    return zf_solver_create_impl(out, desc, opt, stream, h);
}

extern "C" int zf_solver_create_sparse_responses(zf_solver** out, const zf_problem_desc* desc, const zf_spmat* h, int32_t K,
                                                 const zf_options* opt, void* stream) {
    ZF_REQUIRE(out && desc && h && opt, "zf_solver_create_sparse_responses: null argument");
    ZF_REQUIRE(zf_is_sparse_mat(desc->kind),
               "zf_solver_create_sparse_responses: desc->kind must be ZF_PROBLEM_SPARSE_LS_L1 or ZF_PROBLEM_SPARSE_LOGISTIC_L1");
    ZF_REQUIRE(K >= 2 && K <= ZF_SPMM_MAX_K, "zf_solver_create_sparse_responses: K must be 2 .. 16");
    ZF_REQUIRE(desc->world == 1, "zf_solver_create_sparse_responses: not for a sharded solve (world > 1)");
    ZF_REQUIRE(opt->accept_mode == ZF_ACCEPT_REFERENCE, "zf_solver_create_sparse_responses: not with ZF_ACCEPT_REMAINDER or ZF_ACCEPT_RESOLVED");
    return zf_solver_create_impl(out, desc, opt, stream, h, K);
}

extern "C" int zf_solver_destroy(zf_solver* s) {
    if (!s) return ZF_OK;
    (void)hipStreamSynchronize(s->stream);
    zf_solver_free_all(s);
    delete s;
    return ZF_OK;
}

// ... 538 lines not shown
    if (decide_in_launch) {
        zf_launch_op_apply(s->op_plan, s->stream, zf_op_of(s, s->ctl), s->xb[0], s->xb[1], s->xb[2], s->sring.p[0], s->sring.p[1],
                           s->sring.p[2], 1, F);
    } else {
        zf_ring3 xr3 = {{s->xb[0], s->xb[1], s->xb[2]}};
        zf_launch_apply_A(s, s->ctl, xr3, s->sring, 1);
        hipLaunchKernelGGL(zf_resid_x_kernel, dim3(1), dim3(RESID_BLOCK), 0, s->stream, s->ctl, s->sring, 1, d.b,
                           d.scale, m, s->ls_scal + 1);
        zf_launch_finalize(s, false);
    }
    ZF_HIP(hipGetLastError());
    return ZF_OK;
}

static int zf_trial_matrix(zf_solver* s, zf_step_args& a, bool decide_in_launch, hipEvent_t e0, hipEvent_t e1) {
    const zf_problem_desc& d = s->desc;
    const int64_t m = d.m_rows;
    const bool time_whole = (s->sp != nullptr);
    const zf_loss loss = zf_loss_of(s);
    const double gfac = zf_gfac(loss, d.scale);
    if (time_whole && e0) ZF_HIP(hipEventRecord(e0, s->stream));
    const bool wide_resid = (d.kind == ZF_PROBLEM_SPARSE_LS_L1 || (s->o.K > 1 && d.kind == ZF_PROBLEM_LEAST_SQUARES_L1)) &&
                            m > ZF_SPMV_WIDE_RESID_MIN_ROWS;
    if (!zf_launch_loss_y(s->stream, s->ctl, s->sring.p[0], s->sring.p[1], s->sring.p[2], d.b, loss, s->resid, d.scale, m,
                          (int)s->opt.nesterov, s->row_part, s->ls_scal + 0)) {
        if (wide_resid)
            zf_launch_spmv_resid_y(s->stream, s->ctl, s->sring.p[0], s->sring.p[1], s->sring.p[2], d.b, s->resid, d.scale, m,
                                   (int)s->opt.nesterov, s->row_part, s->ls_scal + 0);
        else
            hipLaunchKernelGGL(zf_resid_y_kernel, dim3(1), dim3(RESID_BLOCK), 0, s->stream, s->ctl, s->beta_ring, s->sring, d.b,
                               s->resid, d.scale, m, s->ls_scal + 0, (int)s->opt.nesterov);
    }
    const bool rows = d.world > 1 && d.row_sharded;
    zf_launch_adjoint(zf_mat_of(s), s->stream, s->ctl, s->resid, rows ? s->s_part : s->grad, gfac, s->ws, !rows);
    if (rows) {
        if (s->timing) {
            s->ev_used -= 1;
            if (a.pass_log) s->launches -= 1;
        }
        ZF_HIP(hipGetLastError());
        return ZF_OK;
    }
    a.p0 = s->grad;
    a.p1 = nullptr;
    if (!time_whole && e0) ZF_HIP(hipEventRecord(e0, s->stream));
    zf_launch_trial_kernels(s, a, false);
    if (!time_whole && e1) ZF_HIP(hipEventRecord(e1, s->stream));
    zf_ring3 xr = {{s->xb[0], s->xb[1], s->xb[2]}};
    zf_ring3 sout = s->sring;
    if (d.world > 1) sout = {{s->s_part, s->s_part, s->s_part}};
    zf_launch_apply(zf_mat_of(s), s->stream, s->ctl, xr, sout, 1, s->ws);
    if (d.world == 1) {
        if (!zf_launch_loss_x(s->stream, s->ctl, s->sring.p[0], s->sring.p[1], s->sring.p[2], 1, d.b, loss, d.scale, m,
                              s->row_part + ZF_SPMV_RESID_MAX_CHUNKS, s->ls_scal + 1)) {
            if (wide_resid && s->rem && (s->sp != nullptr))
                zf_launch_spmv_resid_x_rem(s->stream, s->ctl, s->sring.p[0], s->sring.p[1], s->sring.p[2], 1, d.b, d.scale, m,
                                           (int)s->opt.nesterov, 0.0, s->row_part + ZF_SPMV_RESID_MAX_CHUNKS,
                                           s->row_part + 2 * ZF_SPMV_RESID_MAX_CHUNKS, s->ls_scal + 1, s->ls_scal + 2);
            else if (wide_resid)
                zf_launch_spmv_resid_x(s->stream, s->ctl, s->sring.p[0], s->sring.p[1], s->sring.p[2], 1, d.b, d.scale, m,
                                       s->row_part + ZF_SPMV_RESID_MAX_CHUNKS, s->ls_scal + 1);
            else
                zf_launch_resid_x(s);
        }
        zf_launch_finalize(s, decide_in_launch);
    }
    if (time_whole && e1) ZF_HIP(hipEventRecord(e1, s->stream));
    ZF_HIP(hipGetLastError());
    return ZF_OK;
}

static int zf_launch_trial(zf_solver* s, bool decide_in_launch, bool dry = false, bool* done_ahead = nullptr) {
    const zf_problem_desc& d = s->desc;
    zf_step_args a;
    zf_fill_step_args(s, a);
    if (done_ahead) *done_ahead = false;
    hipEvent_t e0 = nullptr, e1 = nullptr;
    if (s->timing && !dry) {
        a.pass_log = s->pass_log;
        a.pass_slot = (int)(s->launches % ZF_PASS_LOG);
        a.pass_tag = (int)(s->launches & 0x7fff) << 16;
        s->launches += 1;
    }
    if (s->timing) {
        if (s->ev_used == s->ev_pool.size()) {
            hipEvent_t x, y;
            ZF_HIP(hipEventCreate(&x));
            ZF_HIP(hipEventCreate(&y));
            s->ev_pool.emplace_back(x, y);
        }
        e0 = s->ev_pool[s->ev_used].first;
        e1 = s->ev_pool[s->ev_used].second;
        s->ev_used++;
    }
    if (d.kind == ZF_PROBLEM_DIAG_QUAD_L1) return zf_trial_diag(s, a, decide_in_launch, dry, done_ahead, e0, e1);
    if (zf_small_open(s) && !dry && decide_in_launch) return zf_trial_ls_small(s, a, e0, e1);
    if (d.kind == ZF_PROBLEM_BLUR_HAAR_L1) return zf_trial_op(s, a, decide_in_launch, e0, e1);
    return zf_trial_matrix(s, a, decide_in_launch, e0, e1);
}

extern "C" int zf_solver_enqueue_trial_finish(zf_solver* s) {
    ZF_REQUIRE(s && s->initialised, "zf_solver_enqueue_trial_finish: solver not initialised");
    const zf_problem_desc& d = s->desc;
    if (d.kind != ZF_PROBLEM_LEAST_SQUARES_L1 || d.world == 1) return ZF_OK;
    const int64_t m = d.m_rows;
    if (d.row_sharded) {
        const int64_t n = d.n;
        zf_ring3 g3 = {{s->grad, s->grad, s->grad}};
        hipLaunchKernelGGL(zf_sum_parts_kernel, dim3(zf_grid_for(n)), dim3(ZF_BLOCK), 0, s->stream, nullptr, s->s_all,
                           (int)d.world, n, g3, -1);
        zf_step_args a;
        zf_fill_step_args(s, a);
        a.p0 = s->grad;
        a.p1 = nullptr;
        zf_launch_trial_kernels(s, a, false);
        zf_ring3 xr = {{s->xb[0], s->xb[1], s->xb[2]}};
        zf_launch_apply(zf_mat_of(s), s->stream, s->ctl, xr, s->sring, 1, s->ws);
        zf_launch_resid_x(s);
        zf_launch_finalize(s, false);
        ZF_HIP(hipGetLastError());
        return ZF_OK;
    }
    hipLaunchKernelGGL(zf_sum_parts_kernel, dim3(zf_grid_for(m)), dim3(ZF_BLOCK), 0, s->stream, s->ctl, s->s_all,
                       (int)d.world, m, s->sring, 1);
    zf_launch_resid_x(s);
    zf_launch_finalize(s, false);
    ZF_HIP(hipGetLastError());
    return ZF_OK;
}

static int zf_init_ls_tail(zf_solver* s) {
    const zf_problem_desc& d = s->desc;
    const int64_t n = d.n, m = d.m_rows;
    zf_ring3 s0 = {{s->sring.p[0], s->sring.p[0], s->sring.p[0]}};
    ZF_HIP(hipMemcpyAsync(s->sring.p[2], s->sring.p[0], sizeof(double) * m, hipMemcpyDeviceToDevice, s->stream));
    const bool own_rows = zf_launch_loss_x(s->stream, nullptr, s0.p[0], s0.p[0], s0.p[0], -1, d.b, zf_loss_of(s), d.scale, m, s->row_part,
                                           s->ls_scal + 1);
    if (!own_rows && m > (int64_t)1 << 18) {
        const int wgs = zf_grid_for(m / 8);
        hipLaunchKernelGGL(zf_resid_x_wide_kernel, dim3(wgs), dim3(ZF_BLOCK), 0, s->stream, s0.p[0], d.b, m, s->partials);
        hipLaunchKernelGGL(zf_resid_x_finish_kernel, dim3(1), dim3(RESID_BLOCK), 0, s->stream, s->partials, wgs, d.scale, s->ls_scal + 1);
    } else if (!own_rows) {
        hipLaunchKernelGGL(zf_resid_x_kernel, dim3(1), dim3(RESID_BLOCK), 0, s->stream, nullptr, s0, -1, d.b, d.scale,
                           m, s->ls_scal + 1);
    }
    const int g = zf_grid_for(n);
    if (s->o.l2 > 0.0) {
        if (s->box)
            hipLaunchKernelGGL(zf_eval_enet_kernel<true>, dim3(g), dim3(ZF_BLOCK), 0, s->stream, s->xb[0], d.lam, 0.5 * s->o.l2, d.box_lo,
                               d.box_hi, n, s->partials);
        else
            hipLaunchKernelGGL(zf_eval_enet_kernel<false>, dim3(g), dim3(ZF_BLOCK), 0, s->stream, s->xb[0], d.lam, 0.5 * s->o.l2, d.box_lo,
                               d.box_hi, n, s->partials);
    } else if (s->o.pf) {
        if (s->box)
            hipLaunchKernelGGL(zf_eval_pf_kernel<true>, dim3(g), dim3(ZF_BLOCK), 0, s->stream, s->xb[0], s->o.pf, d.box_lo, d.box_hi, n, s->partials);
        else
            hipLaunchKernelGGL(zf_eval_pf_kernel<false>, dim3(g), dim3(ZF_BLOCK), 0, s->stream, s->xb[0], s->o.pf, d.box_lo, d.box_hi, n, s->partials);
    } else if (s->box)
        hipLaunchKernelGGL((zf_eval_kernel<false, true>), dim3(g), dim3(ZF_BLOCK), 0, s->stream, s->xb[0], nullptr,
                           nullptr, d.box_lo, d.box_hi, n, s->partials);
    else
        hipLaunchKernelGGL((zf_eval_kernel<false, false>), dim3(g), dim3(ZF_BLOCK), 0, s->stream, s->xb[0], nullptr,
                           nullptr, d.box_lo, d.box_hi, n, s->partials);
    zf_init_args I;
    I.partials = s->partials;
    I.nblocks = g;
    I.f_scale = 0.0;
    I.lam = zf_g_scale(s);
    I.f_ext = s->ls_scal + 1;
    I.pack = s->pack_local;
    I.contribute_g = (d.world == 1 || !d.row_sharded || d.rank == 0) ? 1 : 0;
    hipLaunchKernelGGL(zf_init_finalize_kernel, dim3(1), dim3(ZF_FIN_BLOCK), 0, s->stream, I);
    ZF_HIP(hipGetLastError());
    if (d.world == 1)
        ZF_HIP(hipMemcpyAsync(s->pack_all, s->pack_local, sizeof(double) * ZF_PACK_LEN, hipMemcpyDeviceToDevice,
                              s->stream));
    return ZF_OK;
}

extern "C" int zf_solver_svec_ptrs(zf_solver* s, double** s_part_dev, double** s_all_dev) {
    ZF_REQUIRE(s && s_part_dev && s_all_dev, "zf_solver_svec_ptrs: null argument");
    *s_part_dev = s->s_part;
    *s_all_dev = s->s_all;
    return ZF_OK;
}

extern "C" int zf_solver_set_svec_buffers(zf_solver* s, double* s_part_dev, double* s_all_dev) {
    ZF_REQUIRE(s && s_part_dev && s_all_dev, "zf_solver_set_svec_buffers: null argument");
    ZF_REQUIRE(!s->initialised, "zf_solver_set_svec_buffers: call before zf_solver_enqueue_init");
    ZF_REQUIRE(s->desc.kind == ZF_PROBLEM_LEAST_SQUARES_L1 && s->desc.world > 1,
               "zf_solver_set_svec_buffers: only for sharded least squares (m doubles per rank for column blocks, n for row blocks)");
    if (s->own_svec) {
        if (s->s_part) (void)hipFree(s->s_part);
        if (s->s_all) (void)hipFree(s->s_all);
    }
    s->own_svec = false;
    s->s_part = s_part_dev;
    s->s_all = s_all_dev;
    return ZF_OK;
}

extern "C" int zf_solver_enqueue_init(zf_solver* s, const double* x0_dev) {
    ZF_REQUIRE(s && x0_dev, "zf_solver_enqueue_init: null argument");
    s->init_enqueued = true;
    s->shadow_valid = false;
    const zf_problem_desc& d = s->desc;
    const int64_t n = d.n;
    ZF_HIP(hipMemcpyAsync(s->xb[0], x0_dev, sizeof(double) * n, hipMemcpyDeviceToDevice, s->stream));
    ZF_HIP(hipMemcpyAsync(s->xb[s->ring - 1], x0_dev, sizeof(double) * n, hipMemcpyDeviceToDevice, s->stream));
    zf_control c;
    memset(&c, 0, sizeof(c));
    c.lr = s->opt.lr;
    c.tol = s->opt.tol;
    c.tol_internal = s->opt.tol_internal;
    c.decay_rate = s->opt.decay_rate;
    c.max_iter = s->opt.max_iter;
    c.max_backtrack = s->opt.max_backtrack_iter;
    c.status = (s->opt.max_backtrack_iter == 0) ? ZF_BACKTRACK_FAILED : ZF_RUNNING;
    c.cur = 0;
    c.nesterov = s->opt.nesterov;
    c.deprecated = s->opt.deprecated;
    c.accept_mode = s->accept_mode;
    c.need_grad = 1;
    c.world = d.world;
    c.ring_size = s->ring;
    c.sub_iters = s->sub;
    c.prev = s->ring - 1;
    c.lag = 0;
    c.pend_status = 0;
    ZF_HIP(hipMemcpyAsync(s->ctl, &c, sizeof(c), hipMemcpyHostToDevice, s->stream));
    ZF_HIP(hipStreamSynchronize(s->stream));
    zf_init_args I;
    I.partials = s->partials;
    I.lam = d.lam;
    I.pack = s->pack_local;
    I.f_ext = nullptr;
    I.contribute_g = 1;
    const int g = zf_grid_for(n);
    I.nblocks = g;
    if (d.kind == ZF_PROBLEM_DIAG_QUAD_L1) {
        I.f_scale = 0.5;
        if (s->box)
            hipLaunchKernelGGL((zf_eval_kernel<true, true>), dim3(g), dim3(ZF_BLOCK), 0, s->stream, s->xb[0],
                               d.d, d.c, d.box_lo, d.box_hi, n, s->partials);
        else
            hipLaunchKernelGGL((zf_eval_kernel<true, false>), dim3(g), dim3(ZF_BLOCK), 0, s->stream, s->xb[0],
                               d.d, d.c, d.box_lo, d.box_hi, n, s->partials);
    } else {
        zf_ring3 xr = {{s->xb[0], s->xb[0], s->xb[0]}};
        double* dst = (d.world > 1 && !d.row_sharded) ? s->s_part : s->sring.p[0];
        zf_ring3 s0 = {{dst, dst, dst}};
        zf_launch_apply_A(s, nullptr, xr, s0, -1);
        ZF_HIP(hipGetLastError());
        if (d.world > 1 && !d.row_sharded) return ZF_OK;
        return zf_init_ls_tail(s);
    }
    hipLaunchKernelGGL(zf_init_finalize_kernel, dim3(1), dim3(ZF_FIN_BLOCK), 0, s->stream, I);
    ZF_HIP(hipGetLastError());
    if (d.world == 1)
        ZF_HIP(hipMemcpyAsync(s->pack_all, s->pack_local, sizeof(double) * ZF_PACK_LEN,
                              hipMemcpyDeviceToDevice, s->stream));
    return ZF_OK;
}

static bool zf_fused_small_runs(const zf_solver* s) { return zf_small_open(s) && !s->comm && s->own_packs; }

extern "C" int zf_solver_restore(zf_solver* s, const double* xk_dev, const double* xprev_dev,
                                 const zf_control* saved, int64_t saved_bytes) {
    ZF_REQUIRE(s && xk_dev && xprev_dev && saved, "zf_solver_restore: null argument");
    ZF_REQUIRE(saved_bytes == (int64_t)sizeof(zf_control),
               "zf_solver_restore: saved_bytes differs from zf_sizeof_control() (a control block of another ABI version)");
    const zf_problem_desc& d = s->desc;
    ZF_REQUIRE(d.kind == ZF_PROBLEM_DIAG_QUAD_L1 || d.world == 1,
               "zf_solver_restore: sharded least squares is not supported");
    ZF_REQUIRE(saved->nit >= 0 && saved->lr > 0.0, "zf_solver_restore: implausible control block");
    const int64_t n = d.n;
    s->shadow_valid = false;
    ZF_HIP(hipMemcpyAsync(s->xb[0], xk_dev, sizeof(double) * n, hipMemcpyDeviceToDevice, s->stream));
    ZF_HIP(hipMemcpyAsync(s->xb[s->ring - 1], xprev_dev, sizeof(double) * n, hipMemcpyDeviceToDevice, s->stream));
    zf_control c = *saved;
    c.tol = s->opt.tol;
    c.tol_internal = s->opt.tol_internal;
    c.decay_rate = s->opt.decay_rate;
    c.max_iter = s->opt.max_iter;
    c.max_backtrack = s->opt.max_backtrack_iter;
    c.nesterov = s->opt.nesterov;
    c.deprecated = s->opt.deprecated;
    c.accept_mode = s->accept_mode;
    c.cur = 0;
    c.prev = s->ring - 1;
    c.ring_size = s->ring;
    c.world = d.world;
    c.need_grad = 1;
    ZF_REQUIRE(saved->lag >= 0 && saved->lag <= 2 * s->sub - 2,
               "zf_solver_restore: the saved state lags more iterations than this chain length can replay "
               "(zf_solver_flush before taking the snapshot)");
    c.sub_iters = s->sub;
    c.pass_seq = 0;
    if (c.status == ZF_MAXITER && c.nit < c.max_iter) c.status = ZF_RUNNING;
    if (s->pack_all)
        ZF_HIP(hipMemsetAsync(s->pack_all, 0, sizeof(double) * ZF_PACK_LEN * s->sub * d.world, s->stream));
    ZF_HIP(hipMemcpyAsync(s->ctl, &c, sizeof(c), hipMemcpyHostToDevice, s->stream));
    ZF_HIP(hipStreamSynchronize(s->stream));
    if (zf_has_margins(d.kind)) {
        const int at[2] = {0, 2};
        for (int k = 0; k < 2; ++k) {
            double* xsrc = s->xb[at[k]];
            double* dst = s->sring.p[at[k]];
            if (zf_fused_small_runs(s) && saved->nit >= 1 + k) {
                const dim3 gr((unsigned)((d.m_rows + ZF_WAVES - 1) / ZF_WAVES));
                hipLaunchKernelGGL(zf_ls_small_apply_kernel, gr, dim3(ZF_BLOCK), 0, s->stream, d.A, xsrc, dst, d.m_rows, d.n);
                continue;
            }
            zf_ring3 xr = {{xsrc, xsrc, xsrc}};
            zf_ring3 so = {{dst, dst, dst}};
            zf_launch_apply_A(s, nullptr, xr, so, -1);
        }
        ZF_HIP(hipGetLastError());
    }
    s->initialised = true;
    return ZF_OK;
}

extern "C" int zf_solver_get_x_prev(zf_solver* s, double* x_host, int64_t count) {
    ZF_REQUIRE(s && x_host, "zf_solver_get_x_prev: null argument");
    ZF_REQUIRE(count >= s->desc.n, "zf_solver_get_x_prev: the host buffer holds fewer than n doubles");
    zf_control c;
    ZF_HIP(hipMemcpyAsync(&c, s->ctl, sizeof(c), hipMemcpyDeviceToHost, s->stream));
    ZF_HIP(hipStreamSynchronize(s->stream));
    ZF_HIP(hipMemcpyAsync(x_host, s->xb[c.prev], sizeof(double) * s->desc.n, hipMemcpyDeviceToHost, s->stream));
    ZF_HIP(hipStreamSynchronize(s->stream));
    return ZF_OK;
}

extern "C" int zf_solver_enqueue_init_finish(zf_solver* s) {
    ZF_REQUIRE(s, "zf_solver_enqueue_init_finish: null solver");
    const zf_problem_desc& d = s->desc;
    if (d.kind != ZF_PROBLEM_LEAST_SQUARES_L1 || d.world == 1 || d.row_sharded) return ZF_OK;
    zf_ring3 s0 = {{s->sring.p[0], s->sring.p[0], s->sring.p[0]}};
    hipLaunchKernelGGL(zf_sum_parts_kernel, dim3(zf_grid_for(d.m_rows)), dim3(ZF_BLOCK), 0, s->stream, nullptr,
                       s->s_all, (int)d.world, d.m_rows, s0, -1);
    ZF_HIP(hipGetLastError());
    return zf_init_ls_tail(s);
}

extern "C" int zf_solver_enqueue_init_commit(zf_solver* s) {
    ZF_REQUIRE(s, "zf_solver_enqueue_init_commit: null solver");
    const int f_repl = (s->desc.kind == ZF_PROBLEM_LEAST_SQUARES_L1 && !s->desc.row_sharded) ? 1 : 0;
    hipLaunchKernelGGL(zf_init_commit_kernel, dim3(1), dim3(64), 0, s->stream, s->ctl, s->pack_all, f_repl,
                       s->sub * ZF_PACK_LEN);
    ZF_HIP(hipGetLastError());
    s->initialised = true;
    return ZF_OK;
}

extern "C" int zf_solver_set_beta(zf_solver* s, int64_t first, const double* beta_host, int64_t count) {
    ZF_REQUIRE(s && beta_host, "zf_solver_set_beta: null argument");
    ZF_REQUIRE(first >= 0 && count >= 0 && count <= ZF_RING, "zf_solver_set_beta: bad range");
    int64_t done = 0;
    while (done < count) {
// ... 46 lines not shown
    zf_option_store(&next, opt, a);
    double *part = nullptr, *slab = nullptr;
    if (zf_options_need_loss_part(B, next) && !s->loss_part) ZF_HIP(hipMalloc(&part, sizeof(double) * 2 * ZF_SPMV_RESID_MAX_CHUNKS));
    int slices = s->ws.slices;
    int64_t rows_per_slice = s->ws.rows_per_slice;
    if (zf_is_dense_mat(B.kind)) zf_view_slices(zf_mat_of(s, next), &slices, &rows_per_slice);
    const hipError_t e = slices > s->ws.slices ? hipMalloc(&slab, sizeof(double) * slices * B.n) : hipSuccess;
    if (e != hipSuccess) {
        if (part) (void)hipFree(part);
        return zf_fail(ZF_ERR_HIP, "%s: the slab of the column sweep: %s", ZF_OPTION_RULES[opt].entry, hipGetErrorString(e));
    }
    if (part) {
        if (s->row_part) (void)hipFree(s->row_part);
        s->row_part = part;
        s->loss_part = true;
    }
    if (slab) {
        if (s->ws.slab) (void)hipFree(s->ws.slab);
        s->ws.slab = slab;
    }
    s->ws.slices = slices;
    s->ws.rows_per_slice = rows_per_slice;
    s->o = next;
    s->small_shape = zf_options_small_open(B, next);
    return ZF_OK;
}

extern "C" int zf_solver_set_l2(zf_solver* s, double l2) {
    ZF_REQUIRE(s, "zf_solver_set_l2: null argument");
    return zf_solver_set_option(s, ZF_OPT_L2, zf_option_arg{l2, nullptr, 0});
}
extern "C" int zf_solver_set_penalty_factors(zf_solver* s, const double* p_dev) {
    ZF_REQUIRE(s, "zf_solver_set_penalty_factors: null argument");
    return zf_solver_set_option(s, ZF_OPT_PF, zf_option_arg{0.0, p_dev, 0});
}
extern "C" int zf_solver_set_huber(zf_solver* s, double delta) {
    ZF_REQUIRE(s, "zf_solver_set_huber: null argument");
    return zf_solver_set_option(s, ZF_OPT_HUBER, zf_option_arg{delta, nullptr, 0});
}
extern "C" int zf_solver_set_poisson(zf_solver* s) {
    ZF_REQUIRE(s, "zf_solver_set_poisson: null argument");
    return zf_solver_set_option(s, ZF_OPT_POISSON, zf_option_arg{0.0, nullptr, 0});
}
extern "C" int zf_solver_set_multinomial(zf_solver* s) {
    ZF_REQUIRE(s, "zf_solver_set_multinomial: null argument");
    return zf_solver_set_option(s, ZF_OPT_MULTINOMIAL, zf_option_arg{0.0, nullptr, 0});
}
extern "C" int zf_solver_set_row_weights(zf_solver* s, const double* w_dev) {
    ZF_REQUIRE(s, "zf_solver_set_row_weights: null argument");
    return zf_solver_set_option(s, ZF_OPT_ROWW, zf_option_arg{0.0, w_dev, 0});
}
extern "C" int zf_solver_set_matrix_f32(zf_solver* s, const float* A32_dev) {
    ZF_REQUIRE(s, "zf_solver_set_matrix_f32: null argument");
    return zf_solver_set_option(s, ZF_OPT_A32, zf_option_arg{0.0, A32_dev, 0});
}
extern "C" int zf_solver_set_responses(zf_solver* s, int32_t K) {
    ZF_REQUIRE(s, "zf_solver_set_responses: null argument");
    return zf_solver_set_option(s, ZF_OPT_K, zf_option_arg{0.0, nullptr, (int)K});
}

extern "C" int zf_solver_launch_counts(zf_solver* s, int64_t* out, int64_t count) {
    ZF_REQUIRE(s && out, "zf_solver_launch_counts: null argument");
    ZF_REQUIRE(count >= 2, "zf_solver_launch_counts: the output holds fewer than 2 values");
    out[0] = s->steps_issued;
    out[1] = s->kernels_issued;
    if (count >= 4) out[2] = out[3] = 0;
    if (count >= 6) {
        out[4] = s->ra_passes;
        out[5] = s->ra_ahead;
    }
    if (count >= 8) {
        out[6] = s->ra_timeouts;
        out[7] = s->ra_voids;
    }
    if (count >= 10) {
        out[8] = s->ah_passes;
        out[9] = s->ah_voids;
    }
    if (count >= 11) out[10] = s->ra_off ? 1 : 0;
    if (count >= 12) out[11] = s->second_voids;
    return ZF_OK;
}

extern "C" int zf_solver_ls_plan(zf_solver* s, int64_t* out, int64_t count) {
    ZF_REQUIRE(s && out, "zf_solver_ls_plan: null argument");
    ZF_REQUIRE(count >= 4, "zf_solver_ls_plan: the output holds fewer than 4 values");
    out[0] = out[1] = out[2] = out[3] = 0;
    if (s->desc.kind == ZF_PROBLEM_BLUR_HAAR_L1) {
        const zf_op_plan& pl = s->op_plan;
        out[0] = pl.ty;
        out[1] = pl.sep ? 1 : 0;
        out[2] = pl.persist ? 1 : 0;
        out[3] = (pl.fuse_prox && !s->hist) ? 1 : 0;
        return ZF_OK;
    }
    if (zf_is_sparse_mat(s->desc.kind)) {
        out[0] = 5;
        out[1] = s->sp->A.lanes;
        out[2] = s->sp->At.lanes;
        out[3] = s->sp->A.nsplit + s->sp->At.nsplit;
        if (count >= 6) {
            out[4] = s->o.K;
            out[5] = 0;
        }
        return ZF_OK;
    }
    if (!zf_is_dense_mat(s->desc.kind)) return ZF_OK;
    const zf_matview V = zf_mat_of(s);
    const bool odd = V.n % 2 != 0;
    out[0] = zf_small_open(s) ? 1 : V.mfma ? 2 : odd ? 4 : 3;
    out[1] = zf_small_open(s) ? 1 : odd ? 3 : 2;
    if (V.A32) {
        const int w = zf_f32_width(V.n);
        out[0] = w == 4 ? 6 : w == 2 ? 7 : 8;
        out[1] = w == 4 ? 4 : w == 2 ? 5 : 6;
    }
    if (V.k > 1) {
        out[0] = odd ? 10 : 9;
        out[1] = odd ? 8 : 7;
    }
    out[2] = s->ws.slices;
    out[3] = s->ws.rows_per_slice;
    if (count >= 6) {
        out[4] = V.k;
        out[5] = V.k > 1 ? zf_mr_rows_per_wg(V.k) : 0;
    }
    return ZF_OK;
}

extern "C" int zf_solver_sub_iters(zf_solver* s, int32_t* sub_iters) {
    ZF_REQUIRE(s && sub_iters, "zf_solver_sub_iters: null argument");
    *sub_iters = s->sub;
    return ZF_OK;
}

extern "C" int zf_solver_set_max_iter(zf_solver* s, int64_t max_iter) {
    ZF_REQUIRE(s && s->initialised, "zf_solver_set_max_iter: solver not initialised");
    ZF_REQUIRE(max_iter >= 1, "zf_solver_set_max_iter: max_iter must be >= 1");
    if (s->shadow_valid) {
        zf_control& c = s->shadow;
        c.max_iter = max_iter;
        if (c.status == ZF_MAXITER && c.nit < max_iter) c.status = ZF_RUNNING;
        if (c.pend_status == ZF_MAXITER && c.nit < max_iter) c.pend_status = 0;
    }
    s->opt.max_iter = max_iter;
    hipLaunchKernelGGL(zf_set_max_iter_kernel, dim3(1), dim3(64), 0, s->stream, s->ctl, max_iter);
    ZF_HIP(hipGetLastError());
    return ZF_OK;
}

extern "C" int zf_solver_flush(zf_solver* s) {
    ZF_REQUIRE(s && s->initialised, "zf_solver_flush: solver not initialised");
    if (s->shadow_valid) {
        zf_control& c = s->shadow;
        if (c.status == ZF_RUNNING && c.lag > 0 && c.pend_status == 0) c.pend_status = ZF_PEND_FLUSH;
    }
    hipLaunchKernelGGL(zf_flush_kernel, dim3(1), dim3(64), 0, s->stream, s->ctl);
    ZF_HIP(hipGetLastError());
    return ZF_OK;
}

extern "C" int zf_solver_set_comm(zf_solver* s, zf_comm* comm) {
    ZF_REQUIRE(s && comm, "zf_solver_set_comm: null argument");
    int32_t rank = 0, world = 1;
    int rc = zf_comm_info(comm, &rank, &world);
    if (rc) return rc;
// ... 67 lines not shown
        ZF_REQUIRE(s->desc.world == 1, "zf_solver_enqueue_init_all: world > 1 needs zf_solver_set_comm");
    }
    return zf_solver_enqueue_init_commit(s);
}

extern "C" int zf_solver_enqueue_steps(zf_solver* s, int64_t steps) {
    ZF_REQUIRE(s && s->initialised, "zf_solver_enqueue_steps: solver not initialised");
    ZF_REQUIRE(s->desc.world == 1 || s->comm, "zf_solver_enqueue_steps: world > 1 needs zf_solver_set_comm "
                                              "(or the caller's own trial / gather / decide sequence)");
    ZF_REQUIRE(steps >= 0 && steps <= ZF_RING, "zf_solver_enqueue_steps: steps must be in [0, ZF_RING]");
    for (int64_t k = 0; k < steps; ++k) {
        int rc;
        if (!s->comm) {
            if ((rc = zf_launch_trial(s, true))) return rc;
            continue;
        }
        bool ahead = false;
        s->chunk_last = k + 1 == steps;
        rc = zf_launch_trial(s, false, false, &ahead);
        s->chunk_last = false;
        if (rc) return rc;
        if (ahead) continue;
        if ((rc = zf_gather_svec(s))) return rc;
        if ((rc = zf_solver_enqueue_trial_finish(s))) return rc;
        if ((rc = zf_gather_packs(s, s->sub, nullptr))) return rc;
        if ((rc = zf_solver_enqueue_decide(s))) return rc;
    }
    if (s->stream2) return zf_ra_join(s);
    return ZF_OK;
}

static void zf_set_tiles(zf_solver* s, int tiles) {
    if (tiles < 1) tiles = 1;
    if (tiles > ZF_MAX_TILES_PER_WG) tiles = ZF_MAX_TILES_PER_WG;
    s->tiles = tiles;
    s->grid = (int)((s->ntiles + tiles - 1) / tiles);
}

static int zf_tiles_for(int64_t ntiles) {
    constexpr int64_t SLOTS = 512;
    if (ntiles <= SLOTS) return 1;
    const int t_lo = ntiles < 4096 ? 1 : 8, t_hi = ntiles < 4096 ? 8 : ZF_MAX_TILES_PER_WG;
    int best_t = t_lo;
    double best_cost = 0.0;
    for (int t = t_lo; t <= t_hi; ++t) {
        const int64_t wgs = (ntiles + t - 1) / t;
        const int64_t rounds = (wgs + SLOTS - 1) / SLOTS;
        const double cost = (double)rounds * ((double)t + 0.3);
        if (t == t_lo || cost < best_cost - 1e-9) {
            best_cost = cost;
            best_t = t;
        }
    }
    return best_t;
}

extern "C" int zf_solver_autotune(zf_solver* s, int32_t* chosen_tiles) {
    ZF_REQUIRE(s && s->initialised, "zf_solver_autotune: solver not initialised");
    if (s->env.tiles_per_wg > 0) zf_set_tiles(s, s->env.tiles_per_wg);
    else if (s->desc.kind == ZF_PROBLEM_DIAG_QUAD_L1) zf_set_tiles(s, zf_tiles_for(s->ntiles));
    else zf_set_tiles(s, 1);
    if (chosen_tiles) *chosen_tiles = s->tiles;
    return ZF_OK;
}

extern "C" int zf_solver_pack_ptrs(zf_solver* s, double** pack_local_dev, double** pack_all_dev) {
    ZF_REQUIRE(s && pack_local_dev && pack_all_dev, "zf_solver_pack_ptrs: null argument");
    *pack_local_dev = s->pack_local;
    *pack_all_dev = s->pack_all;
    return ZF_OK;
}

extern "C" int zf_solver_set_pack_buffers(zf_solver* s, double* pack_local_dev, double* pack_all_dev) {
    ZF_REQUIRE(s && pack_local_dev && pack_all_dev, "zf_solver_set_pack_buffers: null argument");
    ZF_REQUIRE(!s->initialised, "zf_solver_set_pack_buffers: call before zf_solver_enqueue_init");
    if (s->pack_local && s->own_packs) (void)hipFree(s->pack_local);
    if (s->pack_all && s->own_packs) (void)hipFree(s->pack_all);
    s->own_packs = false;
    s->pack_local = pack_local_dev;
    s->pack_all = pack_all_dev;
    return ZF_OK;
}

static int zf_collect_timing(zf_solver* s, bool log_in_mail = false) {
    if (!log_in_mail && s->ev_used > 0) {
        const size_t off = ZF_CTL_SLOT + ZF_TRACE_BYTES;
        ZF_HIP(hipMemcpyAsync(s->mail + off, s->ctl_trace + off, sizeof(int) * ZF_PASS_LOG, hipMemcpyDeviceToHost, s->stream));
        ZF_HIP(hipStreamSynchronize(s->stream));
    }
    const bool have_log = s->ev_used > 0 && s->ev_used <= (size_t)ZF_PASS_LOG &&
                          s->launches - s->first_uncollected == (int64_t)s->ev_used;
    const int* log = reinterpret_cast<const int*>(s->mail + ZF_CTL_SLOT + ZF_TRACE_BYTES);
    for (size_t k = 0; k < s->ev_used; ++k) {
        float ms = 0.f;
        ZF_HIP(hipEventElapsedTime(&ms, s->ev_pool[k].first, s->ev_pool[k].second));
        s->ms_total += ms;
        s->ms_count += 1;
        if (have_log) {
            const int64_t launch = s->first_uncollected + (int64_t)k;
            const int entry = log[launch % ZF_PASS_LOG];
            if (entry < 0 || (entry >> 16) != (int)(launch & 0x7fff)) continue;
            const int shape = entry & 0xffff;
            if (shape == 0) continue;
            if (s->records.size() < 65536) s->records.emplace_back(shape, ms);
            const int nf = shape & 31, lag = (shape >> 5) & 31, cnt = (shape >> 10) & 63;
            if (lag == 0 && nf == s->sub) {
                s->ms_full += ms;
                s->n_full += cnt > 0 ? cnt : 1;
            } else {
                s->ms_part += ms;
                s->n_part += 1;
                s->fresh_part += nf;
                s->lag_part += lag;
            }
        }
    }
    s->first_uncollected = s->launches;
    s->ev_used = 0;
    for (size_t k = 0; k < s->xev_used; ++k) {
        float ms = 0.f;
        ZF_HIP(hipEventElapsedTime(&ms, s->xev_pool[k].first, s->xev_pool[k].second));
        s->xms_total += ms;
        s->xms_count += 1;
    }
    s->xev_used = 0;
    return ZF_OK;
}

extern "C" int zf_solver_pass_records(zf_solver* s, double* out, int64_t cap_pairs, int64_t* count) {
    ZF_REQUIRE(out && count && cap_pairs >= 0, "zf_solver_pass_records: bad argument");
    ZF_REQUIRE(s, "zf_solver_pass_records: null solver");
    ZF_HIP(hipStreamSynchronize(s->stream));
    int rc = zf_collect_timing(s);
    if (rc) return rc;
    int64_t k = 0;
    for (; k < (int64_t)s->records.size() && k < cap_pairs; ++k) {
        out[2 * k] = (double)s->records[k].first;
        out[2 * k + 1] = (double)s->records[k].second;
    }
    *count = k;
    s->records.clear();
    return ZF_OK;
}

extern "C" int zf_solver_exchange_stats(zf_solver* s, double* out, int64_t count) {
    ZF_REQUIRE(out && count >= 2, "zf_solver_exchange_stats: needs a buffer of >= 2 doubles");
    ZF_REQUIRE(s, "zf_solver_exchange_stats: null solver");
    ZF_HIP(hipStreamSynchronize(s->stream));
    int rc = zf_collect_timing(s);
    if (rc) return rc;
    out[0] = s->xms_count ? s->xms_total / (double)s->xms_count : 0.0;
    out[1] = (double)s->xms_count;
    s->xms_total = 0.0;
    s->xms_count = 0;
    return ZF_OK;
}

extern "C" int zf_solver_poll(zf_solver* s, zf_control* ctl_host, int64_t ctl_bytes, double* trace_host,
                              int64_t trace_bytes) {
    ZF_REQUIRE(s && ctl_host, "zf_solver_poll: null argument");
    ZF_REQUIRE(ctl_bytes >= (int64_t)sizeof(zf_control),
               "zf_solver_poll: ctl_bytes is smaller than zf_sizeof_control() (host built against another ABI version?)");
    ZF_REQUIRE(!trace_host || trace_bytes >= (int64_t)(sizeof(double) * ZF_RING * ZF_TRACE_COLS),
               "zf_solver_poll: trace_bytes is smaller than ZF_RING * ZF_TRACE_COLS doubles");
    const size_t trace_len = ZF_TRACE_BYTES;
    const bool with_log = s->ev_used > 0;
    const size_t want = with_log ? ZF_MAIL_BYTES : trace_host ? ZF_CTL_SLOT + trace_len : ZF_CTL_SLOT;
    ZF_HIP(hipMemcpyAsync(s->mail, s->ctl_trace, want, hipMemcpyDeviceToHost, s->stream));
    ZF_HIP(hipStreamSynchronize(s->stream));
    memcpy(ctl_host, s->mail, sizeof(zf_control));
    if (trace_host) memcpy(trace_host, s->mail + ZF_CTL_SLOT, trace_len);
    {
        const int64_t rej = ctl_host->total_trials - ctl_host->nit;
        s->careful = s->shadow_valid ? (rej != s->polled_rejections) : (rej != 0);
        s->polled_rejections = rej;
        s->shadow = *ctl_host;
        s->shadow_valid = true;
        s->steps_since_poll = 0;
        const unsigned* st = reinterpret_cast<const unsigned*>(s->mail + ZF_STATS_OFF);
        s->ra_timeouts = st[0];
        s->ra_voids = st[1];
        s->ah_voids = st[2];
        s->second_voids = st[3];
        if (s->ra_timeouts > 0) s->ra_off = true;
    }
    return zf_collect_timing(s, with_log);
}

extern "C" int zf_solver_x_dev(zf_solver* s, const double** x_dev) {
    ZF_REQUIRE(s && x_dev, "zf_solver_x_dev: null argument");
    zf_control c;
    ZF_HIP(hipMemcpyAsync(&c, s->ctl, sizeof(c), hipMemcpyDeviceToHost, s->stream));
    ZF_HIP(hipStreamSynchronize(s->stream));
    *x_dev = s->xb[c.cur];
    return ZF_OK;
}

extern "C" int zf_solver_get_x(zf_solver* s, double* x_host, int64_t count) {
    ZF_REQUIRE(s && x_host, "zf_solver_get_x: null argument");
    ZF_REQUIRE(count >= s->desc.n, "zf_solver_get_x: the host buffer holds fewer than n doubles");
    const double* xd = nullptr;
    int rc = zf_solver_x_dev(s, &xd);
    if (rc) return rc;
    ZF_HIP(hipMemcpyAsync(x_host, xd, sizeof(double) * s->desc.n, hipMemcpyDeviceToHost, s->stream));
    ZF_HIP(hipStreamSynchronize(s->stream));
    return ZF_OK;
}

extern "C" int zf_solver_set_timing(zf_solver* s, int32_t enabled) {
    ZF_REQUIRE(s, "zf_solver_set_timing: null solver");
    s->timing = enabled != 0;
    return ZF_OK;
}

extern "C" int zf_solver_pass_stats(zf_solver* s, double* out, int64_t count) {
    ZF_REQUIRE(s && out && count >= 4, "zf_solver_pass_stats: needs a buffer of >= 4 doubles");
    ZF_HIP(hipStreamSynchronize(s->stream));
    int rc = zf_collect_timing(s);
    if (rc) return rc;
    out[0] = s->n_full ? s->ms_full / (double)s->n_full : 0.0;
    out[1] = (double)s->n_full;
    out[2] = s->n_part ? s->ms_part / (double)s->n_part : 0.0;
    out[3] = (double)s->n_part;
    s->ms_full = s->ms_part = 0.0;
    s->n_full = s->n_part = 0;
    s->fresh_part = s->lag_part = 0;
    s->ms_total = 0.0;
    s->ms_count = 0;
    return ZF_OK;
}

extern "C" int zf_solver_pass_stats_ex(zf_solver* s, double* out, int64_t count) {
    ZF_REQUIRE(s && out && count >= 6, "zf_solver_pass_stats_ex: needs a buffer of >= 6 doubles");
    ZF_HIP(hipStreamSynchronize(s->stream));
    int rc = zf_collect_timing(s);
    if (rc) return rc;
    out[4] = (double)s->fresh_part;
    out[5] = (double)s->lag_part;
    return zf_solver_pass_stats(s, out, 4);
}

extern "C" int zf_solver_trial_kernel_ms(zf_solver* s, double* avg_ms, int64_t* launches) {
    ZF_REQUIRE(s && avg_ms && launches, "zf_solver_trial_kernel_ms: null argument");
    ZF_HIP(hipStreamSynchronize(s->stream));
    int rc = zf_collect_timing(s);
    if (rc) return rc;
    *launches = s->ms_count;
    *avg_ms = s->ms_count ? s->ms_total / (double)s->ms_count : 0.0;
    s->ms_total = 0.0;
    s->ms_count = 0;
    s->ms_full = s->ms_part = 0.0;
    s->n_full = s->n_part = 0;
// ... 383 lines not shown
```

### zfista_amd/engine.py

```python
from __future__ import annotations

import ctypes as C
import os

import numpy as np

from . import _lib


def momentum_factors(count: int, ratio, state=None):
    a, b = ratio
    t_prev = 1 if state is None else state
    out = np.empty(count, dtype=np.float64)
    for j in range(count):
        t_next = np.sqrt(t_prev**2 - a * t_prev + b) + 0.5
        out[j] = (t_prev - 1) / t_next
        t_prev = t_next
    return out, t_prev


def gather_packs(pack_all, pack_local, group):
    import torch.distributed as dist

    if pack_local.is_cuda and dist.get_backend(group) == "gloo":
# ... 181 lines not shown
            self.trial_finish()
            self._gather()
            self.enqueue_decide()

    def set_history(self, ring_dev_ptr: int, cap_slots: int, stride: int):
        _lib.check(self.lib.zf_solver_set_history(self.handle, C.c_void_p(ring_dev_ptr), int(cap_slots), int(stride)),
                   "set_history")

    def flush(self):
        _lib.check(self.lib.zf_solver_flush(self.handle), "flush")
        self.enqueue(1)

    def get_x_prev(self) -> np.ndarray:
        out = np.empty(self.n, dtype=np.float64)
        _lib.check(self.lib.zf_solver_get_x_prev(self.handle, C.c_void_p(_lib.ptr(out)), out.size), "get_x_prev")
        return out

    def restore(self, xk_dev_ptr: int, xprev_dev_ptr: int, ctl):
        _lib.check(self.lib.zf_solver_restore(self.handle, C.c_void_p(xk_dev_ptr), C.c_void_p(xprev_dev_ptr),
                                              C.byref(ctl), C.sizeof(ctl)), "restore")
        t = C.c_int32(1)
        _lib.check(self.lib.zf_solver_autotune(self.handle, C.byref(t)), "geometry")
        self.tiles_per_wg = int(t.value)

    def set_max_iter(self, max_iter: int):
        _lib.check(self.lib.zf_solver_set_max_iter(self.handle, int(max_iter)), "set_max_iter")

    def poll(self):
        _lib.check(self.lib.zf_solver_poll(self.handle, C.byref(self.ctl), C.sizeof(self.ctl),
                                           C.c_void_p(_lib.ptr(self.trace)), self.trace.nbytes), "poll")
        return self.ctl, self.trace

    def get_x(self) -> np.ndarray:
        out = np.empty(self.n, dtype=np.float64)
        _lib.check(self.lib.zf_solver_get_x(self.handle, C.c_void_p(_lib.ptr(out)), out.size), "get_x")
        return out

    def duality_gap(self) -> np.ndarray:
        out = np.zeros(10 if self.l2 > 0 else 8)
        _lib.check(self.lib.zf_solver_duality_gap(self.handle, C.c_void_p(_lib.ptr(out)), out.size), "zf_solver_duality_gap")
        return out

    def x_dev_ptr(self) -> int:
        p = C.c_void_p()
        _lib.check(self.lib.zf_solver_x_dev(self.handle, C.byref(p)))
        return p.value

    def trial_kernel_ms(self):
        ms, cnt = C.c_double(0.0), C.c_int64(0)
        _lib.check(self.lib.zf_solver_trial_kernel_ms(self.handle, C.byref(ms), C.byref(cnt)))
        return ms.value, cnt.value

    def pass_stats(self):
        out = np.zeros(4)
        _lib.check(self.lib.zf_solver_pass_stats(self.handle, C.c_void_p(_lib.ptr(out)), out.size))
        return (out[0], int(out[1])), (out[2], int(out[3]))

    def launch_counts(self):
        out = np.zeros(2, dtype=np.int64)
        _lib.check(self.lib.zf_solver_launch_counts(self.handle, C.c_void_p(_lib.ptr(out)), out.size))
        return int(out[0]), int(out[1])

    def ls_plan(self):
        out = np.zeros(4, dtype=np.int64)
        _lib.check(self.lib.zf_solver_ls_plan(self.handle, C.c_void_p(_lib.ptr(out)), out.size))
        return tuple(int(v) for v in out)

    def responses_plan(self):
        out = np.zeros(6, dtype=np.int64)
        _lib.check(self.lib.zf_solver_ls_plan(self.handle, C.c_void_p(_lib.ptr(out)), out.size))
        return int(out[4]), int(out[5])

    def runahead_counts(self):
        out = np.zeros(6, dtype=np.int64)
        _lib.check(self.lib.zf_solver_launch_counts(self.handle, C.c_void_p(_lib.ptr(out)), out.size))
        return int(out[4]), int(out[5])

    def ahead_report(self):
        out = np.zeros(12, dtype=np.int64)
        _lib.check(self.lib.zf_solver_launch_counts(self.handle, C.c_void_p(_lib.ptr(out)), out.size))
        return dict(runahead=int(out[4]), runahead_overlapped=int(out[5]), timeouts=int(out[6]), void=int(out[7]),
                    ahead=int(out[8]), ahead_void=int(out[9]), runahead_off=bool(out[10]), second_void=int(out[11]))

    def pass_stats_ex(self):
        out = np.zeros(6)
        _lib.check(self.lib.zf_solver_pass_stats_ex(self.handle, C.c_void_p(_lib.ptr(out)), out.size))
        return (out[0], int(out[1])), (out[2], int(out[3])), (int(out[4]), int(out[5]))

    def pass_records(self, cap=65536):
        out = np.zeros(2 * cap)
        cnt = C.c_int64(0)
        _lib.check(self.lib.zf_solver_pass_records(self.handle, C.c_void_p(_lib.ptr(out)), cap, C.byref(cnt)))
        rec = []
        for k in range(cnt.value):
            shape = int(out[2 * k])
            rec.append(((shape >> 5) & 31, shape & 31, (shape >> 10) & 63, float(out[2 * k + 1])))
        return rec

    def exchange_stats(self):
        out = np.zeros(2)
        _lib.check(self.lib.zf_solver_exchange_stats(self.handle, C.c_void_p(_lib.ptr(out)), out.size))
        return out[0], int(out[1])

    def close(self):
        if getattr(self, "handle", None):
            self.lib.zf_solver_destroy(self.handle)
            self.handle = None

    def __del__(self):
        try:
            self.close()
        except Exception:
            pass
```

Before: 11400.

## Poll solver state through a mapped-memory mirror kernel instead of memcpy+sync

Replaces the per-poll device-to-host hipMemcpyAsync plus hipStreamSynchronize with a small mirror kernel that writes the control block, new trace rows and log slots into coherent mapped host memory and publishes a sequence token. The host then spins on that token, so it avoids a full stream sync and a large copy on each poll. The trace is copied incrementally, and timing for the diagonal problem uses in-kernel wall_clock64 stamps instead of events. The cost is an extra kernel launch per poll, host busy-waiting, and more complex fallback paths.

```diff
diff --git a/include/zfista_hip.h b/include/zfista_hip.h
--- a/include/zfista_hip.h
+++ b/include/zfista_hip.h
@@ -177,6 +177,7 @@
                       int64_t saved_bytes );
 int zf_solver_trial_kernel_ms(zf_solver* s, double* avg_ms, int64_t* launches);
 int zf_solver_launch_counts(zf_solver* s, int64_t* out, int64_t count );
+int zf_solver_poll_counts(zf_solver* s, int64_t* out, int64_t count );
 int zf_solver_ls_plan(zf_solver* s, int64_t* out, int64_t count );
 int zf_solver_pass_stats(zf_solver* s, double* out, int64_t count );
 int zf_solver_pass_stats_ex(zf_solver* s, double* out, int64_t count );
diff --git a/zfista_amd/_lib.py b/zfista_amd/_lib.py
--- a/zfista_amd/_lib.py
+++ b/zfista_amd/_lib.py
@@ -155,6 +155,7 @@
     "zf_solver_exchange_stats": (C.c_int, [_P, _P, C.c_int64]),
     "zf_solver_pass_records": (C.c_int, [_P, _P, C.c_int64, C.POINTER(C.c_int64)]),
     "zf_solver_launch_counts": (C.c_int, [_P, _P, C.c_int64]),
+    "zf_solver_poll_counts": (C.c_int, [_P, _P, C.c_int64]),
     "zf_solver_ls_plan": (C.c_int, [_P, _P, C.c_int64]),
     "zf_host_grad_step": (C.c_int, [_P, _P, _P, C.c_double, C.c_int64]),
     "zf_host_model_terms": (C.c_int, [_P, _P, _P, C.c_int64, _P]),
@@ -303,7 +304,8 @@
                 "ZF_COMM", "ZF_MO_COMM", "ZF_MO_LAUNCH_AHEAD", "ZF_MO_SPIN_LIMIT", "ZF_RCCL_LIB", "ZF_DUAL_SOLVER",
                 "ZF_FORCE_SPLIT", "ZF_LIB_PATH", "ZF_BENCH_BACKEND",
                 "ZF_RUNAHEAD", "ZF_RUNAHEAD_SPIN_LIMIT", "ZF_PASS_SEQ_START", "ZF_AHEAD",
-                "ZF_AHEAD_UNSHARDED", "ZF_ACCEPT", "ZF_OP_SEPARABLE", "ZF_OP_FUSE_PROX", "ZF_OP_PERSIST", "ZF_RUNAHEAD_SHARDED")
+                "ZF_AHEAD_UNSHARDED", "ZF_ACCEPT", "ZF_OP_SEPARABLE", "ZF_OP_FUSE_PROX", "ZF_OP_PERSIST", "ZF_RUNAHEAD_SHARDED",
+                "ZF_POLL_COPY")
 
 
 def env_overrides() -> dict:
diff --git a/zfista_amd/csrc/zf_common.h b/zfista_amd/csrc/zf_common.h
--- a/zfista_amd/csrc/zf_common.h
+++ b/zfista_amd/csrc/zf_common.h
@@ -37,6 +37,7 @@
     bool op_fuse_prox;
     bool op_persist;
     long long mo_spin_limit;
+    bool poll_copy;
 };
 zf_env zf_env_read();
 
diff --git a/zfista_amd/csrc/zf_kernels_step.h b/zfista_amd/csrc/zf_kernels_step.h
--- a/zfista_amd/csrc/zf_kernels_step.h
+++ b/zfista_amd/csrc/zf_kernels_step.h
@@ -218,6 +218,7 @@
     int* pass_log;
     int pass_slot;
     int pass_tag;
+    unsigned long long* pass_clk;
     double* hist;
     int64_t hist_cap;
     int64_t hist_stride;
@@ -246,6 +247,17 @@
 };
 
 ZF_HD inline int zf_log_shape(int lag, int nf, int passes) { return (nf & 31) | ((lag & 31) << 5) | ((passes & 63) << 10); }
+__device__ __forceinline__ void zf_clk_stamp(const zf_step_args& A, int which) {
+    if (A.pass_clk) A.pass_clk[2 * A.pass_slot + which] = (unsigned long long)wall_clock64();
+}
+__device__ __forceinline__ unsigned long long zf_clk_take(const zf_step_args& A) {
+    unsigned long long t = 0;
+    if (A.pass_clk && blockIdx.x == 0) t = (unsigned long long)wall_clock64();
+    return t;
+}
+__device__ __forceinline__ void zf_clk_put(const zf_step_args& A, unsigned long long t0) {
+    if (t0 != 0 && threadIdx.x == 0) A.pass_clk[2 * A.pass_slot] = t0;
+}
 
 struct zf_finalize_args {
     const double* blk_part;
@@ -518,6 +530,7 @@
     if constexpr (RA) {
         if (!A.decide) {
             if (t == 0 && A.pass_log) A.pass_log[A.pass_slot] = A.pass_tag | zf_log_shape(0, LEN, 0);
+            if (t == 0) zf_clk_stamp(A, 1);
             return;
         }
         constexpr int CW = (int)(sizeof(zf_control) / 8);
@@ -559,12 +572,14 @@
         asm volatile("s_waitcnt vmcnt(0)" ::: "memory");
         if (t == 0)
             __hip_atomic_store(A.ra_word, ((unsigned long long)(unsigned)A.pass_seq << 32) | good, __ATOMIC_RELAXED, __HIP_MEMORY_SCOPE_AGENT);
+        if (t == 0) zf_clk_stamp(A, 1);
         return;
     }
     if (A.decide) {
         zf_decide_pass_wave(A.ctl_rw, s_pack, pk, A.trace, A.beta_ring, t, LSTR, s_pre);
         if (t == 0) A.ctl_rw->pass_seq = A.pass_seq;
     }
+    if (t == 0) zf_clk_stamp(A, 1);
 }
 
 struct zf_ahead_check {
@@ -657,6 +672,7 @@
         zf_decide_ahead(A.ctl_rw, s_pack, pk, A.trace, A.beta_ring, t, LSTR, s_pre, H, true, A.ra_word, A.ra_stats, A.pass_log,
                         A.pass_slot, A.pass_tag);
     }
+    if (t == 0) zf_clk_stamp(A, 1);
 }
 
 __device__ __forceinline__ unsigned long long zf_uniform_u64(unsigned long long v) {
@@ -687,7 +703,8 @@
 template <bool GRAD_INLINE, bool NESTEROV, bool BOX, bool NT, int S, int MODE, bool HIST, int SP = S, bool COH = false, bool RES = false,
           bool ENET = false, bool PF = false>
 __device__ __forceinline__ double zf_trial_body(const zf_step_args& A, double* lds, const zf_pass_head& HD, const int lag,
-                                                const int nf, zf_d2* stage = nullptr, const double l2 = 0.0) {
+                                                const int nf, zf_d2* stage = nullptr, const double l2 = 0.0,
+                                                unsigned long long* clk0 = nullptr) {
     constexpr bool FULL = (MODE == 0);
     static_assert(!RES || GRAD_INLINE, "resolved differences f(x+) - f(y): the separable problem");
     static_assert(!ENET || (!GRAD_INLINE && S == 1 && MODE == 0 && !COH), "elastic net: single trials on a gradient vector");
@@ -729,6 +746,7 @@
         lr_i = zf_readlane_f64(rp_lr, i);
         tau_i = zf_readlane_f64(rp_tau, i);
     };
+    if (clk0) *clk0 = zf_clk_take(A);
     int first, second;
     zf_free_bufs(cur, prev, ring, &first, &second);
     const double* __restrict__ xk = A.xb[cur];
@@ -1084,6 +1102,7 @@
                           : PART != 1 ? zf_uses_glds<S, PART == 0 ? 0 : 2, HIST, GRAD_INLINE>()
                                       : (S >= 16 && zf_uses_glds<S / 2, 1, HIST, GRAD_INLINE, S>());
     __shared__ zf_d2 stage[GLDS ? ZF_GLDS_NST * ZF_GLDS_STAGE_UNITS : 1];
+    unsigned long long clk0 = 0;
     if constexpr (AHEAD) {
         if (A.ra_need != 0) {
             const unsigned long long W = __hip_atomic_load(A.ra_word, __ATOMIC_RELAXED, __HIP_MEMORY_SCOPE_AGENT);
@@ -1108,7 +1127,8 @@
         HA.beta_next = NESTEROV ? A.beta_ring[HA.nit % ZF_RING] : 0.0;
         constexpr int LEN = PART == 3 ? L : S;
         if (A.pass_log && blockIdx.x == 0 && threadIdx.x == 0) A.pass_log[A.pass_slot] = A.pass_tag | zf_log_shape(0, LEN, 0);
-        const double va = zf_trial_body<GRAD_INLINE, NESTEROV, BOX, NT, LEN, 0, HIST, S, false, RES>(A, lds, HA, 0, LEN, stage);
+        const double va = zf_trial_body<GRAD_INLINE, NESTEROV, BOX, NT, LEN, 0, HIST, S, false, RES>(A, lds, HA, 0, LEN, stage, 0.0, &clk0);
+        zf_clk_put(A, clk0);
         if (threadIdx.x < S * ZF_NPART) A.blk_part[(int64_t)blockIdx.x * (S * ZF_NPART) + threadIdx.x] = va;
         return;
     }
@@ -1117,7 +1137,9 @@
     const zf_pass_head HD = zf_head_of(A.ctl);
     if constexpr (S == 1) {
         if (A.pass_log && blockIdx.x == 0 && threadIdx.x == 0) A.pass_log[A.pass_slot] = A.pass_tag | zf_log_shape(0, 1, 0);
-        zf_pass_finish<S>(A, zf_trial_body<GRAD_INLINE, NESTEROV, BOX, NT, S, 0, HIST, S, false, RES>(A, lds, HD, 0, 1));
+        const double v1 = zf_trial_body<GRAD_INLINE, NESTEROV, BOX, NT, S, 0, HIST, S, false, RES>(A, lds, HD, 0, 1, nullptr, 0.0, &clk0);
+        zf_clk_put(A, clk0);
+        zf_pass_finish<S>(A, v1);
     } else {
         const int lag = A.ctl->lag;
         const int nf = zf_fresh_len(A.ctl);
@@ -1129,21 +1151,22 @@
         if (A.pass_log && blockIdx.x == 0 && threadIdx.x == 0) A.pass_log[A.pass_slot] = A.pass_tag | zf_log_shape(lag, nf, 0);
         double v;
         if constexpr (PART == 0) {
-            v = zf_trial_body<GRAD_INLINE, NESTEROV, BOX, NT, S, 0, HIST, S, false, RES>(A, lds, HD, 0, S, stage);
+            v = zf_trial_body<GRAD_INLINE, NESTEROV, BOX, NT, S, 0, HIST, S, false, RES>(A, lds, HD, 0, S, stage, 0.0, &clk0);
         } else if constexpr (PART == 3) {
-            v = zf_trial_body<GRAD_INLINE, NESTEROV, BOX, NT, L, 0, HIST, S, false, RES>(A, lds, HD, 0, L, stage);
+            v = zf_trial_body<GRAD_INLINE, NESTEROV, BOX, NT, L, 0, HIST, S, false, RES>(A, lds, HD, 0, L, stage, 0.0, &clk0);
         } else if constexpr (PART == 2) {
             const int nf_opaque = __builtin_amdgcn_readfirstlane(nf);
-            v = zf_trial_body<GRAD_INLINE, NESTEROV, BOX, NT, S, 2, HIST, S, false, RES>(A, lds, HD, lag, nf_opaque, stage);
+            v = zf_trial_body<GRAD_INLINE, NESTEROV, BOX, NT, S, 2, HIST, S, false, RES>(A, lds, HD, lag, nf_opaque, stage, 0.0, &clk0);
         } else if constexpr (S >= 16) {
             constexpr int SS = S / 2;
-            if (lag == 0 && nf == SS) v = zf_trial_body<GRAD_INLINE, NESTEROV, BOX, NT, SS, 0, HIST, S, false, RES>(A, lds, HD, 0, SS, stage);
-            else if (nf == SS) v = zf_trial_body<GRAD_INLINE, NESTEROV, BOX, NT, SS, 1, HIST, S, false, RES>(A, lds, HD, lag, SS, stage);
-            else v = zf_trial_body<GRAD_INLINE, NESTEROV, BOX, NT, SS, 2, HIST, S, false, RES>(A, lds, HD, lag, nf, stage);
+            if (lag == 0 && nf == SS) v = zf_trial_body<GRAD_INLINE, NESTEROV, BOX, NT, SS, 0, HIST, S, false, RES>(A, lds, HD, 0, SS, stage, 0.0, &clk0);
+            else if (nf == SS) v = zf_trial_body<GRAD_INLINE, NESTEROV, BOX, NT, SS, 1, HIST, S, false, RES>(A, lds, HD, lag, SS, stage, 0.0, &clk0);
+            else v = zf_trial_body<GRAD_INLINE, NESTEROV, BOX, NT, SS, 2, HIST, S, false, RES>(A, lds, HD, lag, nf, stage, 0.0, &clk0);
         } else {
-            if (nf == S) v = zf_trial_body<GRAD_INLINE, NESTEROV, BOX, NT, S, 1, HIST, S, false, RES>(A, lds, HD, lag, S);
-            else v = zf_trial_body<GRAD_INLINE, NESTEROV, BOX, NT, S, 2, HIST, S, false, RES>(A, lds, HD, lag, nf);
-        }
+            if (nf == S) v = zf_trial_body<GRAD_INLINE, NESTEROV, BOX, NT, S, 1, HIST, S, false, RES>(A, lds, HD, lag, S, nullptr, 0.0, &clk0);
+            else v = zf_trial_body<GRAD_INLINE, NESTEROV, BOX, NT, S, 2, HIST, S, false, RES>(A, lds, HD, lag, nf, nullptr, 0.0, &clk0);
+        }
+        zf_clk_put(A, clk0);
         zf_pass_finish<S>(A, v);
     }
 }
@@ -1180,6 +1203,7 @@
     __shared__ int s_go;
     zf_pass_head HD = A.ra_head;
     const int b = (int)blockIdx.x, G = (int)gridDim.x;
+    const unsigned long long clk0 = zf_clk_take(A);
     if (A.ra_wait == 0) {
         const zf_control* c = A.ctl;
         const bool same = c->status == ZF_RUNNING && c->pend_status == 0 && c->lag == 0 && c->nit == HD.nit && c->lr == HD.lr &&
@@ -1231,6 +1255,7 @@
     HD.beta_next = NESTEROV ? zf_uniform_f64(A.beta_ring[HD.nit % ZF_RING]) : 0.0;
     double v = 0.0;
     if (run) v = zf_trial_body<true, NESTEROV, BOX, NT, LEN, 0, false, S, true, RES>(A, lds, HD, 0, LEN, stage);
+    zf_clk_put(A, clk0);
     zf_step_args T = A;
     T.ctl = A.ctl_rw;
     T.ctl_rw = &s_ctl;
diff --git a/zfista_amd/csrc/zf_solver.hip b/zfista_amd/csrc/zf_solver.hip
--- a/zfista_amd/csrc/zf_solver.hip
+++ b/zfista_amd/csrc/zf_solver.hip
@@ -1,4 +1,6 @@
 #include <algorithm>
+#include <atomic>
+#include <chrono>
 #include <cstring>
 #include <map>
 #include <mutex>
@@ -292,13 +294,26 @@
     double* hist = nullptr;
     int64_t hist_cap = 0, hist_stride = 0;
     zf_gap_ws gap = {nullptr, nullptr, nullptr, nullptr};
+    unsigned long long* pass_clk = nullptr;
+    size_t clk_used = 0;
+    double clk_khz = 0.0;
+    char* mail_dev = nullptr;
+    unsigned long long poll_seq = 0;
+    int64_t mail_nit = 0;
+    bool mail_trace_ok = false;
+    int64_t poll_fallbacks = 0;
+    int64_t poll_mirrored = 0;
 };
 constexpr int ZF_PASS_LOG = 4096;
 constexpr size_t ZF_CTL_SLOT = (sizeof(zf_control) + 255) / 256 * 256;
 constexpr size_t ZF_STATS_OFF = ZF_CTL_SLOT - 32;
 static_assert(sizeof(zf_control) <= ZF_STATS_OFF, "the run-ahead counters live behind the control block, inside its slot");
 constexpr size_t ZF_TRACE_BYTES = sizeof(double) * ZF_RING * ZF_TRACE_COLS;
-constexpr size_t ZF_MAIL_BYTES = ZF_CTL_SLOT + ZF_TRACE_BYTES + sizeof(int) * ZF_PASS_LOG;
+constexpr size_t ZF_LOG_OFF = ZF_CTL_SLOT + ZF_TRACE_BYTES;
+constexpr size_t ZF_COPY_BYTES = ZF_LOG_OFF + sizeof(int) * ZF_PASS_LOG;
+constexpr size_t ZF_CLK_OFF = ZF_COPY_BYTES;
+constexpr size_t ZF_TOKEN_OFF = ZF_CLK_OFF + 2 * sizeof(unsigned long long) * ZF_PASS_LOG;
+constexpr size_t ZF_MAIL_BYTES = ZF_TOKEN_OFF + 128;
 
 static int zf_tiles_for(int64_t ntiles);
 constexpr bool ZF_AHEAD_UNSHARDED_DEFAULT = false;
@@ -321,6 +336,7 @@
     v.op_fuse_prox = !((e = getenv("ZF_OP_FUSE_PROX")) && atoi(e) == 0);
     v.op_persist = !((e = getenv("ZF_OP_PERSIST")) && atoi(e) == 0);
     v.mo_spin_limit = (e = getenv("ZF_MO_SPIN_LIMIT")) ? atoll(e) : 0;
+    v.poll_copy = (e = getenv("ZF_POLL_COPY")) && atoi(e) != 0;
     return v;
 }
 
@@ -599,7 +615,17 @@
     s->ra_stats = reinterpret_cast<unsigned*>(s->ctl_trace + ZF_STATS_OFF);
     ZF_TRY(hipMemsetAsync(s->ctl_trace, 0, ZF_CTL_SLOT, s->stream));
     ZF_TRY(hipMemsetAsync(s->pass_log, 0xff, sizeof(int) * ZF_PASS_LOG, s->stream));
-    ZF_TRY(hipHostMalloc(&s->mail, ZF_MAIL_BYTES, hipHostMallocDefault));
+    s->pass_clk = reinterpret_cast<unsigned long long*>(s->ctl_trace + ZF_CLK_OFF);
+    ZF_TRY(hipMemsetAsync(s->pass_clk, 0, ZF_TOKEN_OFF - ZF_CLK_OFF, s->stream));
+    ZF_TRY(hipHostMalloc(&s->mail, ZF_MAIL_BYTES, hipHostMallocMapped | hipHostMallocCoherent));
+    memset(s->mail, 0, ZF_MAIL_BYTES);
+    ZF_TRY(hipHostGetDevicePointer(reinterpret_cast<void**>(&s->mail_dev), s->mail, 0));
+    {
+        int dev = 0, khz = 0;
+        ZF_TRY(hipGetDevice(&dev));
+        ZF_TRY(hipDeviceGetAttribute(&khz, hipDeviceAttributeWallClockRate, dev));
+        s->clk_khz = khz > 0 ? (double)khz : 1e5;
+    }
     ZF_TRY(hipMalloc(&s->beta_ring, sizeof(double) * ZF_RING));
     ZF_TRY(hipMalloc(&s->pack_local, sizeof(double) * ZF_PACK_LEN * s->sub));
     ZF_TRY(hipMalloc(&s->pack_all, sizeof(double) * ZF_PACK_LEN * s->sub * desc->world));
@@ -1304,7 +1330,11 @@
         a.pass_tag = (int)(s->launches & 0x7fff) << 16;
         s->launches += 1;
     }
-    if (s->timing) {
+    const bool by_clock = s->timing && !dry && d.kind == ZF_PROBLEM_DIAG_QUAD_L1;
+    if (by_clock) {
+        a.pass_clk = s->pass_clk;
+        s->clk_used++;
+    } else if (s->timing) {
         if (s->ev_used == s->ev_pool.size()) {
             hipEvent_t x, y;
             ZF_HIP(hipEventCreate(&x));
@@ -1427,6 +1457,7 @@
     ZF_REQUIRE(s && x0_dev, "zf_solver_enqueue_init: null argument");
     s->init_enqueued = true;
     s->shadow_valid = false;
+    s->mail_trace_ok = false;
     const zf_problem_desc& d = s->desc;
     const int64_t n = d.n;
     ZF_HIP(hipMemcpyAsync(s->xb[0], x0_dev, sizeof(double) * n, hipMemcpyDeviceToDevice, s->stream));
@@ -1499,6 +1530,7 @@
     ZF_REQUIRE(saved->nit >= 0 && saved->lr > 0.0, "zf_solver_restore: implausible control block");
     const int64_t n = d.n;
     s->shadow_valid = false;
+    s->mail_trace_ok = false;
     ZF_HIP(hipMemcpyAsync(s->xb[0], xk_dev, sizeof(double) * n, hipMemcpyDeviceToDevice, s->stream));
     ZF_HIP(hipMemcpyAsync(s->xb[s->ring - 1], xprev_dev, sizeof(double) * n, hipMemcpyDeviceToDevice, s->stream));
     zf_control c = *saved;
@@ -1711,6 +1743,14 @@
     return ZF_OK;
 }
 
+extern "C" int zf_solver_poll_counts(zf_solver* s, int64_t* out, int64_t count) {
+    ZF_REQUIRE(s && out, "zf_solver_poll_counts: null argument");
+    ZF_REQUIRE(count >= 2, "zf_solver_poll_counts: the output holds fewer than 2 values");
+    out[0] = s->poll_mirrored;
+    out[1] = s->poll_fallbacks;
+    return ZF_OK;
+}
+
 extern "C" int zf_solver_ls_plan(zf_solver* s, int64_t* out, int64_t count) {
     ZF_REQUIRE(s && out, "zf_solver_ls_plan: null argument");
     ZF_REQUIRE(count >= 4, "zf_solver_ls_plan: the output holds fewer than 4 values");
@@ -1944,24 +1984,47 @@
     return ZF_OK;
 }
 
+static int zf_copy_slots(zf_solver* s, size_t off, size_t esz, int64_t first, int64_t count) {
+    if (count <= 0) return ZF_OK;
+    if (count >= ZF_PASS_LOG) {
+        ZF_HIP(hipMemcpyAsync(s->mail + off, s->ctl_trace + off, esz * ZF_PASS_LOG, hipMemcpyDeviceToHost, s->stream));
+        return ZF_OK;
+    }
+    const int64_t a = first % ZF_PASS_LOG;
+    const int64_t n1 = std::min<int64_t>(count, ZF_PASS_LOG - a);
+    ZF_HIP(hipMemcpyAsync(s->mail + off + esz * a, s->ctl_trace + off + esz * a, esz * n1, hipMemcpyDeviceToHost, s->stream));
+    if (count > n1) ZF_HIP(hipMemcpyAsync(s->mail + off, s->ctl_trace + off, esz * (count - n1), hipMemcpyDeviceToHost, s->stream));
+    return ZF_OK;
+}
+
 static int zf_collect_timing(zf_solver* s, bool log_in_mail = false) {
-    if (!log_in_mail && s->ev_used > 0) {
-        const size_t off = ZF_CTL_SLOT + ZF_TRACE_BYTES;
-        ZF_HIP(hipMemcpyAsync(s->mail + off, s->ctl_trace + off, sizeof(int) * ZF_PASS_LOG, hipMemcpyDeviceToHost, s->stream));
+    const size_t timed = s->ev_used + s->clk_used;
+    const int64_t logged = s->launches - s->first_uncollected;
+    if (!log_in_mail && timed > 0) {
+        int rc = zf_copy_slots(s, ZF_LOG_OFF, sizeof(int), s->first_uncollected, logged);
+        if (!rc && s->clk_used > 0) rc = zf_copy_slots(s, ZF_CLK_OFF, 2 * sizeof(unsigned long long), s->first_uncollected, logged);
+        if (rc) return rc;
         ZF_HIP(hipStreamSynchronize(s->stream));
     }
-    const bool have_log = s->ev_used > 0 && s->ev_used <= (size_t)ZF_PASS_LOG &&
-                          s->launches - s->first_uncollected == (int64_t)s->ev_used;
-    const int* log = reinterpret_cast<const int*>(s->mail + ZF_CTL_SLOT + ZF_TRACE_BYTES);
-    for (size_t k = 0; k < s->ev_used; ++k) {
+    const bool have_log = timed > 0 && timed <= (size_t)ZF_PASS_LOG && logged == (int64_t)timed;
+    const int* log = reinterpret_cast<const int*>(s->mail + ZF_LOG_OFF);
+    const unsigned long long* clk = reinterpret_cast<const unsigned long long*>(s->mail + ZF_CLK_OFF);
+    for (size_t k = 0; k < timed; ++k) {
+        const int64_t launch = s->first_uncollected + (int64_t)k;
+        const int entry = have_log ? log[launch % ZF_PASS_LOG] : -1;
+        const bool ran = have_log && entry >= 0 && (entry >> 16) == (int)(launch & 0x7fff);
         float ms = 0.f;
-        ZF_HIP(hipEventElapsedTime(&ms, s->ev_pool[k].first, s->ev_pool[k].second));
+        if (s->clk_used > 0) {
+            if (ran && (entry & 0xffff) != 0) {
+                const unsigned long long t0 = clk[2 * (launch % ZF_PASS_LOG)], t1 = clk[2 * (launch % ZF_PASS_LOG) + 1];
+                if (t1 > t0) ms = (float)((double)(t1 - t0) / s->clk_khz);
+            }
+        } else {
+            ZF_HIP(hipEventElapsedTime(&ms, s->ev_pool[k].first, s->ev_pool[k].second));
+        }
         s->ms_total += ms;
         s->ms_count += 1;
-        if (have_log) {
-            const int64_t launch = s->first_uncollected + (int64_t)k;
-            const int entry = log[launch % ZF_PASS_LOG];
-            if (entry < 0 || (entry >> 16) != (int)(launch & 0x7fff)) continue;
+        if (ran) {
             const int shape = entry & 0xffff;
             if (shape == 0) continue;
             if (s->records.size() < 65536) s->records.emplace_back(shape, ms);
@@ -1979,6 +2042,7 @@
     }
     s->first_uncollected = s->launches;
     s->ev_used = 0;
+    s->clk_used = 0;
     for (size_t k = 0; k < s->xev_used; ++k) {
         float ms = 0.f;
         ZF_HIP(hipEventElapsedTime(&ms, s->xev_pool[k].first, s->xev_pool[k].second));
@@ -2018,6 +2082,93 @@
     return ZF_OK;
 }
 
+struct zf_mirror_args {
+    const char* src;
+    char* dst;
+    int64_t trace_from;
+    int with_trace;
+    int with_clk;
+    int64_t slot_first;
+    int slot_count;
+    unsigned long long seq;
+};
+__global__ __launch_bounds__(256) void zf_poll_mirror_kernel(zf_mirror_args M) {
+    const int t = (int)threadIdx.x;
+    const unsigned long long* sw = reinterpret_cast<const unsigned long long*>(M.src);
+    unsigned long long* dw = reinterpret_cast<unsigned long long*>(M.dst);
+    auto put = [&](int64_t w) { __hip_atomic_store(dw + w, sw[w], __ATOMIC_RELAXED, __HIP_MEMORY_SCOPE_SYSTEM); };
+    constexpr int CW = (int)(ZF_CTL_SLOT / 8), RW = ZF_TRACE_COLS;
+    for (int i = t; i < CW; i += 256) put(i);
+    if (M.with_trace) {
+        const int64_t nit = reinterpret_cast<const zf_control*>(M.src)->nit;
+        const int64_t from = M.trace_from, cnt = nit - from;
+        if (from < 0 || cnt < 0 || cnt >= ZF_RING) {
+            for (int i = t; i < ZF_RING * RW; i += 256) put(CW + i);
+        } else {
+            for (int64_t i = t; i < cnt * RW; i += 256) put(CW + ((from + i / RW) % ZF_RING) * RW + i % RW);
+        }
+    }
+    const int* sl = reinterpret_cast<const int*>(M.src + ZF_LOG_OFF);
+    int* dl = reinterpret_cast<int*>(M.dst + ZF_LOG_OFF);
+    for (int k = t; k < M.slot_count; k += 256) {
+        const int64_t slot = (M.slot_first + k) % ZF_PASS_LOG;
+        __hip_atomic_store(dl + slot, sl[slot], __ATOMIC_RELAXED, __HIP_MEMORY_SCOPE_SYSTEM);
+        if (M.with_clk) {
+            put((int64_t)(ZF_CLK_OFF / 8) + 2 * slot);
+            put((int64_t)(ZF_CLK_OFF / 8) + 2 * slot + 1);
+        }
+    }
+    __threadfence_system();
+    __syncthreads();
+    if (t == 0) __hip_atomic_store(dw + ZF_TOKEN_OFF / 8, M.seq, __ATOMIC_RELEASE, __HIP_MEMORY_SCOPE_SYSTEM);
+}
+static_assert(ZF_CTL_SLOT % 8 == 0 && ZF_LOG_OFF % 8 == 0 && ZF_CLK_OFF % 8 == 0 && ZF_TOKEN_OFF % 8 == 0, "the mirror kernel moves 8-byte words");
+
+constexpr double ZF_POLL_SPIN_SECONDS = 2.0;
+static int zf_poll_mirror(zf_solver* s, bool with_trace, int64_t slot_count, bool* seen) {
+    zf_mirror_args M;
+    M.src = s->ctl_trace;
+    M.dst = s->mail_dev;
+    M.trace_from = s->mail_trace_ok ? s->mail_nit : -1;
+    M.with_trace = with_trace ? 1 : 0;
+    M.with_clk = s->clk_used > 0 ? 1 : 0;
+    M.slot_first = s->first_uncollected;
+    M.slot_count = (int)std::min<int64_t>(std::max<int64_t>(slot_count, 0), ZF_PASS_LOG);
+    M.seq = ++s->poll_seq;
+    hipLaunchKernelGGL(zf_poll_mirror_kernel, dim3(1), dim3(256), 0, s->stream, M);
+    ZF_HIP(hipGetLastError());
+    const volatile unsigned long long* token = reinterpret_cast<const volatile unsigned long long*>(s->mail + ZF_TOKEN_OFF);
+    const auto t0 = std::chrono::steady_clock::now();
+    *seen = false;
+    for (unsigned spins = 1;; ++spins) {
+        if (*token == M.seq) {
+            *seen = true;
+            break;
+        }
+#if defined(__x86_64__) || defined(__i386__)
+        __builtin_ia32_pause();
+#endif
+        if ((spins & 1023u) == 0) {
+            const hipError_t q = hipStreamQuery(s->stream);
+            if (q == hipSuccess) {
+                *seen = *token == M.seq;
+                break;
+            }
+            if (q != hipErrorNotReady) return zf_fail(ZF_ERR_HIP, "%s: %s", "hipStreamQuery", hipGetErrorString(q));
+            if (std::chrono::duration<double>(std::chrono::steady_clock::now() - t0).count() > ZF_POLL_SPIN_SECONDS) {
+                ZF_HIP(hipStreamSynchronize(s->stream));
+                *seen = *token == M.seq;
+                break;
+            }
+        }
+    }
+    std::atomic_thread_fence(std::memory_order_acquire);
+    if (*seen) s->poll_mirrored += 1;
+    else s->poll_fallbacks += 1;
+    if (*seen && (s->ev_used > 0 || s->xev_used > 0)) ZF_HIP(hipStreamSynchronize(s->stream));
+    return ZF_OK;
+}
+
 extern "C" int zf_solver_poll(zf_solver* s, zf_control* ctl_host, int64_t ctl_bytes, double* trace_host,
                               int64_t trace_bytes) {
     ZF_REQUIRE(s && ctl_host, "zf_solver_poll: null argument");
@@ -2026,10 +2177,26 @@
     ZF_REQUIRE(!trace_host || trace_bytes >= (int64_t)(sizeof(double) * ZF_RING * ZF_TRACE_COLS),
                "zf_solver_poll: trace_bytes is smaller than ZF_RING * ZF_TRACE_COLS doubles");
     const size_t trace_len = ZF_TRACE_BYTES;
-    const bool with_log = s->ev_used > 0;
-    const size_t want = with_log ? ZF_MAIL_BYTES : trace_host ? ZF_CTL_SLOT + trace_len : ZF_CTL_SLOT;
-    ZF_HIP(hipMemcpyAsync(s->mail, s->ctl_trace, want, hipMemcpyDeviceToHost, s->stream));
-    ZF_HIP(hipStreamSynchronize(s->stream));
+    const bool with_log = s->ev_used + s->clk_used > 0;
+    const int64_t logged = with_log ? s->launches - s->first_uncollected : 0;
+    bool mirrored = false;
+    if (!s->env.poll_copy) {
+        int rc = zf_poll_mirror(s, trace_host != nullptr, logged, &mirrored);
+        if (rc) return rc;
+    }
+    if (!mirrored) {
+        const size_t want = with_log ? ZF_COPY_BYTES : trace_host ? ZF_CTL_SLOT + trace_len : ZF_CTL_SLOT;
+        ZF_HIP(hipMemcpyAsync(s->mail, s->ctl_trace, want, hipMemcpyDeviceToHost, s->stream));
+        if (s->clk_used > 0) {
+            int rc = zf_copy_slots(s, ZF_CLK_OFF, 2 * sizeof(unsigned long long), s->first_uncollected, logged);
+            if (rc) return rc;
+        }
+        ZF_HIP(hipStreamSynchronize(s->stream));
+    }
+    if (trace_host || (!mirrored && with_log)) {
+        s->mail_nit = reinterpret_cast<const zf_control*>(s->mail)->nit;
+        s->mail_trace_ok = true;
+    }
     memcpy(ctl_host, s->mail, sizeof(zf_control));
     if (trace_host) memcpy(trace_host, s->mail + ZF_CTL_SLOT, trace_len);
     {
diff --git a/zfista_amd/engine.py b/zfista_amd/engine.py
--- a/zfista_amd/engine.py
+++ b/zfista_amd/engine.py
@@ -287,6 +287,14 @@
         return dict(runahead=int(out[4]), runahead_overlapped=int(out[5]), timeouts=int(out[6]), void=int(out[7]),
                     ahead=int(out[8]), ahead_void=int(out[9]), runahead_off=bool(out[10]), second_void=int(out[11]))
 
+    def poll_counts(self):
+        out = np.zeros(2, dtype=np.int64)
+        _lib.check(self.lib.zf_solver_poll_counts(self.handle, C.c_void_p(_lib.ptr(out)), out.size))
+        return int(out[0]), int(out[1])
+
+    def poll_fallbacks(self):
+        return self.poll_counts()[1]
+
     def pass_stats_ex(self):
         out = np.zeros(6)
         _lib.check(self.lib.zf_solver_pass_stats_ex(self.handle, C.c_void_p(_lib.ptr(out)), out.size))
```

Measured after the change: 11450, median of 6. About the same (+0.4%).
